# drapado/PINGS

Measured on AMD Instinct MI355X. Metric: raster fwd+bwd Mpix/s @1M Gaussians 1080p, higher is better.
Workload: dtype f32; 1 GPU; surfel rasteriser fwd+bwd, 1000000 Gaussians, 1920x1080, one view per GPU; gaussians=1000000, width=1920, height=1080

## Files before the change

### include/pings_hip.h

```cpp
#ifndef PINGS_HIP_H_
#define PINGS_HIP_H_

#include <stddef.h>
#include <stdint.h>

#if defined(__cplusplus)
#define PINGS_EXTERN_C extern "C"
#else
#define PINGS_EXTERN_C
#endif
#define PINGS_API PINGS_EXTERN_C __attribute__((visibility("default")))

#define PINGS_OK 0
#define PINGS_ERR_ARG 1
#define PINGS_ERR_HIP 2
#define PINGS_ERR_CAPACITY 3


#define PINGS_ABI_VERSION 11
PINGS_API int pings_abi_version(void);
PINGS_API const char* pings_last_error(void);

PINGS_API int pings_prof_enable(int on);
PINGS_API int pings_prof_only(const char* stage);
PINGS_API int pings_prof_report(char* buf, size_t cap);


PINGS_API size_t pings_ssim_partials_count(int planes, int H, int W);

PINGS_API int pings_ssim_forward(const float* img1, const float* img2, int planes, int H, int W,
                                 int train, float* out_mean, float* dm_dmu1,
                                 float* dm_dsigma1_sq, float* dm_dsigma12, float* partials,
                                 void* stream);

PINGS_API int pings_ssim_backward(const float* img1, const float* img2, int planes, int H, int W,
                                  const float* dL_dmean, const float* dm_dmu1,
                                  const float* dm_dsigma1_sq, const float* dm_dsigma12,
                                  float* dL_dimg1, void* stream);


#define PINGS_RASTER_SURFEL 0
#define PINGS_RASTER_3DGS 1
#define PINGS_RASTER_2DGS 2

typedef struct pings_raster_settings {
  int32_t image_height, image_width;
  int32_t mode;
  int32_t front_only;
  double tanfovx, tanfovy;
  double scale_modifier;
  const float* bg;
  const float* viewmatrix;
  const float* projmatrix;
  const float* projmatrix_raw;
  const float* prcppoint;
} pings_raster_settings;

PINGS_API int pings_raster_mark_visible(const float* positions, int N,
                                        const pings_raster_settings* s, uint8_t* present,
                                        void* stream);

PINGS_API size_t pings_raster_geom_bytes(int P, int image_height, int image_width);
PINGS_API size_t pings_raster_binning_bytes(int64_t num_instances, int image_height,
                                            int image_width);
PINGS_API size_t pings_raster_image_bytes(int image_height, int image_width);

PINGS_API int pings_raster_preprocess(const pings_raster_settings* s, int P, const float* means3D,
                                      const float* colors, const float* opacities,
                                      const float* scales, const float* rotations,
                                      void* geom_blob, int32_t* radii, int64_t* num_instances,
                                      int32_t* footprint_class, void* stream);
PINGS_API int pings_raster_preprocess_dyn(const pings_raster_settings* s, int P, const float* means3D,
                                          const float* colors, const float* opacities, const float* scales,
                                          const float* rotations, void* geom_blob, int32_t* radii,
                                          const int32_t* live_rows_dev, int dyn_rows,
                                          const int32_t* const* aux_dev, int aux_words, int32_t* aux_host,
                                          int64_t* num_instances, int32_t* footprint_class, void* stream);

PINGS_API int pings_raster_render(const pings_raster_settings* s, int P, int64_t num_instances,
                                  void* geom_blob, void* binning_blob, void* image_blob,
                                  float* out_color, float* out_normal,
                                  float* out_depth, float* out_alpha, void* per_gaussian,
                                  int footprint_class, void* stream);

PINGS_API size_t pings_raster_tile_sort_bytes(int64_t n, int32_t* block_pairs);
PINGS_API int pings_raster_tile_sort(const void* keys, int64_t n, int key_bytes, int bits, void* keys_sorted,
                                     uint32_t* values, void* scratch, int library, void* stream);

PINGS_API size_t pings_raster_scan_bytes(int64_t n);
PINGS_API int pings_raster_scan_u32(const void* in, int64_t n, int kind, int inclusive, uint32_t* out, void* temp,
                                    size_t temp_bytes, void* stream);

PINGS_API size_t pings_raster_backward_bytes(int P, int64_t num_instances);

PINGS_API int pings_raster_backward(const pings_raster_settings* s, int P, int64_t num_instances,
                                    const float* means3D, const float* colors,
                                    const float* opacities, const float* scales,
                                    const float* rotations, const void* geom_blob,
                                    const void* binning_blob, const void* image_blob,
                                    const float* out_color, const float* out_normal,
                                    const float* out_depth, const float* out_alpha,
                                    const float* dL_dcolor, const float* dL_dnormal,
                                    const float* dL_ddepth, const float* dL_dalpha,
                                    void* bwd_blob, float* dL_dmeans3D, float* dL_dmeans2D,
                                    float* dL_dcolors, float* dL_dopacities, float* dL_dscales,
                                    float* dL_drotations, float* dL_dtau, int footprint_class,
                                    void* stream);

PINGS_API int pings_raster_debug_lists(const void* binning_blob, int64_t num_instances,
                                       int image_height, int image_width, uint32_t* point_list,
                                       uint32_t* ranges_xy, void* stream);
PINGS_API int pings_raster_debug_image(const void* image_blob, int image_height, int image_width,
                                       float* final_T, uint32_t* n_contrib, void* stream);
PINGS_API int pings_raster_debug_occlusion(const void* geom_blob, int P, int image_height, int image_width,
                                           uint32_t* occ_bucket, uint16_t* occ_bsat, int32_t* occ_nb,
                                           void* stream);
PINGS_API int pings_raster_rank_bucket(const int32_t* ranks, int64_t n, int occ_nb, uint32_t nvalid,
                                       uint32_t* buckets);


PINGS_API size_t pings_raster2d_geom_bytes(int P, int image_height, int image_width);
PINGS_API size_t pings_raster2d_binning_bytes(int64_t num_instances, int image_height, int image_width);
PINGS_API size_t pings_raster2d_image_bytes(int image_height, int image_width);

PINGS_API int pings_raster2d_preprocess(const pings_raster_settings* s, int P, const float* means3D,
                                        const float* colors, const float* opacities, const float* scales,
                                        const float* rotations, void* geom_blob, int32_t* radii,
                                        const int32_t* live_rows_dev, int dyn_rows, const int32_t* const* aux_dev,
                                        int aux_words, int32_t* aux_host, int64_t* num_instances, void* stream);

PINGS_API int pings_raster2d_render(const pings_raster_settings* s, int P, int64_t num_instances, void* geom_blob,
                                    void* binning_blob, void* image_blob, float* out_color, float* out_allmap,
                                    void* stream);

PINGS_API size_t pings_raster2d_backward_bytes(int P, int64_t num_instances);

PINGS_API int pings_raster2d_backward(const pings_raster_settings* s, int P, int64_t num_instances,
                                      const float* scales, const float* rotations, const void* geom_blob,
                                      const void* binning_blob, const void* image_blob, const float* dL_dcolor,
                                      const float* dL_dallmap, void* bwd_blob, float* dL_dmeans3D,
                                      float* dL_dmeans2D, float* dL_dcolors, float* dL_dopacities,
                                      float* dL_dscales, float* dL_drotations, void* stream);

PINGS_API int pings_raster2d_debug_lists(const void* binning_blob, int64_t num_instances, int image_height,
                                         int image_width, uint32_t* point_list, uint32_t* ranges_xy, void* stream);
PINGS_API int pings_raster2d_debug_image(const void* image_blob, int image_height, int image_width, float* final_T,
                                         uint32_t* n_contrib, int32_t* median, void* stream);

typedef struct pings_knn_map {
  const int64_t* table;
  int64_t buffer_size;
  const float* neural_points;
  const int32_t* point_ts_create;
  const float* travel_dist;
  int32_t cur_ts;
  int32_t time_filtering;
  float diff_travel_dist_local;
  const uint8_t* free_mask;
  const uint8_t* valid_mask;
  int32_t use_free_mask, use_valid_mask;
  const int64_t* global2local;
  const int32_t* neighbor_dx;
  int32_t K;
  int32_t nn_k;
  float resolution;
  float max_valid_dist2;
  const void* compact;
  uint32_t compact_mask;
  const void* blocks;
  const void* block_records;
  const int32_t* blocks_ok;
  uint32_t block_mask;
} pings_knn_map;

PINGS_API size_t pings_knn_compact_entries(int64_t num_points);
PINGS_API int pings_knn_compact_build(const int64_t* table, int64_t buffer_size, void* compact,
                                      size_t entries, void* stream);

PINGS_API size_t pings_knn_blocks_entries(int64_t num_points);
PINGS_API int pings_knn_blocks_build(const pings_knn_map* m, int64_t num_points, int64_t num_timestamps,
                                     int32_t max_abs_dx, void* blocks, size_t entries, void* records,
                                     int32_t* status, void* stream);

PINGS_API int pings_knn_search(const pings_knn_map* m, const float* queries, int64_t B,
                               int64_t* idx, float* d2, int64_t* nn_counts, int64_t* global_idx,
                               void* stream);
PINGS_API int pings_knn_cells(const pings_knn_map* m, const float* queries, int64_t B, int64_t num_points, float* d2,
                              int64_t* idx, void* stream);

typedef struct pings_qf_tables {
  const float* geo_features;
  const float* color_features;
  int32_t Fg, Fc;
  const float* points;
  const float* orientations;
  const float* certainties;
  int32_t after_pgo;
  int32_t weighted_first;
} pings_qf_tables;

PINGS_API int pings_query_feature_forward(const pings_knn_map* m, const pings_qf_tables* t, const float* queries,
                                          int64_t B, float* geo_out, float* color_out, float* w_out,
                                          int64_t* idx_out, int64_t* gidx_out, int64_t* nn_counts,
                                          float* certainty, float* certainty_accum, const int32_t* query_ts,
                                          int32_t* ts_update, float* n_out, void* stream);
PINGS_API int pings_query_feature_accumulate(const int64_t* idx, const float* w, int64_t n_pairs, float* certainties,
                                             void* stream);

PINGS_API size_t pings_query_feature_scratch_bytes(int64_t B, int nn_k, int64_t rows);
PINGS_API int pings_query_feature_backward(const pings_qf_tables* t, const float* global_points,
                                           const float* queries, int64_t B, int nn_k, const int64_t* idx,
                                           const int64_t* gidx, const float* g_geo, const float* g_color,
                                           const float* g_n, const float* g_w, int64_t rows, void* scratch,
                                           float* g_x, float* g_geo_features, float* g_color_features,
                                           void* stream);

PINGS_API int pings_query_feature_double_backward(
    const pings_qf_tables* t, const float* global_points, const float* queries, int64_t B, int nn_k,
    const int64_t* idx, const int64_t* gidx, const float* g_geo, const float* g_color, const float* g_w,
    const float* gg_x, const float* gg_geo_features, const float* gg_color_features, int64_t rows, void* scratch,
    float* d_g_geo, float* d_g_color, float* d_g_n, float* d_g_w, float* d_x, float* d_geo_features,
    float* d_color_features, void* stream);

PINGS_API size_t pings_rows_scatter_add_scratch_bytes(int64_t n_pairs, int64_t rows);
PINGS_API int pings_rows_scatter_add(const int64_t* dst_row, int64_t n_pairs, const float* src, int64_t ld,
                                     int32_t F, const float* w, const int64_t* src_row, int64_t rows,
                                     void* scratch, float* out, void* stream);
PINGS_API size_t pings_rows_plan_bytes(int64_t n_pairs, int64_t rows);
PINGS_API int pings_rows_plan_build(const int64_t* dst_row, int64_t n_pairs, int64_t rows, void* plan, void* stream);
PINGS_API int pings_rows_plan_apply(const void* plan, int64_t n_pairs, int64_t rows, const float* src, int64_t ld,
                                    int32_t F, const float* w, float* out, void* stream);

typedef struct pings_sdf_decoder {
  const float* W1;
  const float* b1;
  const float* W2;
  const float* b2;
  int32_t hidden;
  int32_t feat_dim;
  float sdf_scale;
  int32_t weighted_first;
} pings_sdf_decoder;

PINGS_API int pings_sdf_forward(const pings_knn_map* m, const pings_sdf_decoder* dec,
                                const float* features, const float* points,
                                const float* orientations, const float* certainties,
                                int32_t after_pgo, const float* queries, int64_t B, float* sdf,
                                float* grad_x, int64_t* nn_counts, float* certainty,
                                int64_t* idx_out, float* w_out, float* sdf_std, int64_t* gidx_out,
                                void* stream);

PINGS_API int pings_sdf_plan(int nn_k, int feat_dim, int hidden, int weighted_first, int order, int misaligned,
                             int32_t* out);

typedef struct pings_color_decoder {
  const float* W1;
  const float* b1;
  const float* W2;
  const float* b2;
  int32_t hidden;
  int32_t feat_dim;
  int32_t channels;
  int32_t weighted_first;
} pings_color_decoder;
PINGS_API int pings_color_forward(const pings_color_decoder* dec, const float* features, int64_t rows,
                                  const float* points, const float* orientations, int32_t after_pgo,
                                  const float* queries, int64_t B, const int64_t* idx, int32_t nn_k, float* color,
                                  float* jac, void* stream);

PINGS_API size_t pings_sdf_backward_scratch_bytes(int64_t B, int nn_k, int feat_dim, int hidden,
                                                  int64_t feature_rows);
// ... 617 lines not shown
```

### pings_amd/_abi.py

```python
from __future__ import annotations

import ctypes as C

ABI_VERSION = 11

RASTER_SURFEL, RASTER_3DGS, RASTER_2DGS = 0, 1, 2
HEAD_COLOR, HEAD_SEMANTIC = 0, 1
REG_SINGULAR, REG_ILL_CONDITIONED, REG_NONFINITE = 1, 2, 4
REG_F_NORMALS, REG_F_DIV_GRAD, REG_F_WEIGHTED = 1, 2, 4
REG_COLOR_PHOTO, REG_COLOR_CONSIST = 1, 2
MC_ALLOW_DEGENERATE, MC_ASCENT = 1, 2
ADAMW_MAX_JOBS, ADAMW_CHUNK = 48, 4096
EVAL_VIEW_RECORD, EVAL_PAIR_RECORD = 9, 12
EVAL_EXTENT = 1
LOOP_MAX_R, LOOP_MAX_S, LOOP_MAX_D = 32, 128, 16
LOOP_MAX_Q, LOOP_MAX_C = 16, 65536
LIDAR_MAX_CAMS, LIDAR_MAX_LIDARS = 8, 8
CAMFRONT_MAX_MAPS, CAMFRONT_TILE_W, CAMFRONT_TILE_H = 32, 128, 32
CAMFRONT_RGB_U8, CAMFRONT_RGB_F32, CAMFRONT_NORMAL, CAMFRONT_DEPTH, CAMFRONT_SKY = 0, 1, 2, 3, 4
CAMFRONT_FIT_RECORD, CAMFRONT_MIN_FIT = 5, 100
CAMFRONT_FULL = 2
TSDF_BLOCK = 8
TSDF_EXTENT, TSDF_TABLE_FULL = 1, 2

# ... 33 lines not shown

class SdfDecoder(C.Structure):
    _fields_ = [("W1", C.c_void_p), ("b1", C.c_void_p), ("W2", C.c_void_p), ("b2", C.c_void_p),
                ("hidden", C.c_int32), ("feat_dim", C.c_int32), ("sdf_scale", C.c_float),
                ("weighted_first", C.c_int32)]


class ColorDecoder(C.Structure):
    _fields_ = [("W1", C.c_void_p), ("b1", C.c_void_p), ("W2", C.c_void_p), ("b2", C.c_void_p),
                ("hidden", C.c_int32), ("feat_dim", C.c_int32), ("channels", C.c_int32),
                ("weighted_first", C.c_int32)]


class MlpJob(C.Structure):
    _fields_ = [("x", C.c_void_p), ("IN", C.c_int32), ("OUT", C.c_int32), ("W1", C.c_void_p), ("b1", C.c_void_p),
                ("W2", C.c_void_p), ("b2", C.c_void_p), ("y", C.c_void_p), ("dL_dy", C.c_void_p), ("dL_dx", C.c_void_p),
                ("dL_dW1", C.c_void_p), ("dL_db1", C.c_void_p), ("dL_dW2", C.c_void_p), ("dL_db2", C.c_void_p)]


class SpawnParams(C.Structure):
    _fields_ = [("n", C.c_int), ("k", C.c_int), ("scale_dim", C.c_int), ("surfel", C.c_int),
                ("color_residual", C.c_int), ("alpha_filter_on", C.c_int), ("scale_filter_on", C.c_int),
                ("displacement_range", C.c_float), ("unit_scale", C.c_float), ("max_scale", C.c_float),
                ("scale_filter_thr", C.c_float)]


class GatherJob(C.Structure):
    _fields_ = [("src", C.c_void_p), ("dst", C.c_void_p), ("row_bytes", C.c_int64), ("rows", C.c_int64)]


class ImageLossParams(C.Structure):
    _fields_ = [("H", C.c_int), ("W", C.c_int), ("v_min", C.c_int), ("v_max", C.c_int), ("depth_min", C.c_float),
                ("depth_max", C.c_float), ("min_accu_alpha", C.c_float), ("inverse_depth", C.c_int),
                ("consist_mode", C.c_int)]


class RegLoopArgs(C.Structure):
    _fields_ = [("n", C.c_int64), ("flags", C.c_int32), ("iter", C.c_int32), ("trace_cap", C.c_int32),
                ("min_grad", C.c_float), ("max_grad", C.c_float), ("max_std", C.c_float), ("gm_dist", C.c_float),
                ("gm_grad", C.c_float), ("lm_lambda", C.c_float)] + \
               [(k, C.c_void_p) for k in ("src", "cur", "sdf", "grad", "std", "mask", "label", "normals", "valid",
                                          "part", "T", "delta", "record", "trace")]


class RegColorArgs(C.Structure):
    _fields_ = [("src_color", C.c_void_p), ("color_pred", C.c_void_p), ("color_jac", C.c_void_p),
                ("channels", C.c_int32), ("mode", C.c_int32), ("photo_weight", C.c_float), ("photo_part", C.c_void_p)]


class GaussLossArgs(C.Structure):
    _fields_ = [("P", C.c_int64), ("Na", C.c_int64), ("cap", C.c_int64), ("R", C.c_int32), ("ncols", C.c_int32),
                ("scale_cols", C.c_int32), ("flags", C.c_int32), ("min_alpha", C.c_float),
                ("contrib_thr", C.c_float), ("shift_range", C.c_float), ("grad_min", C.c_float),
                ("grad_max", C.c_float), ("inv_voxel_pow", C.c_float), ("n_inject", C.c_int64)] + \
               [(n, vp) for n in ("alpha_all", "visible", "contrib", "free_mask", "xyz", "rot", "scale", "alpha", "seed",
                                  "inject_idx", "randn", "keys", "part", "meta", "idx", "normal", "queries", "label",
                                  "sdf", "grad", "nn", "valid", "losses", "counts", "g", "ds", "v", "dn", "dq",
                                  "d_xyz", "d_rot", "d_scale", "d_alpha", "d_alpha_all")]


class SdfHvpArgs(C.Structure):
    _fields_ = [("W1", vp), ("b1", vp), ("W2", vp), ("b2", vp), ("H", C.c_int32), ("F", C.c_int32),
                ("scale", C.c_float), ("after_pgo", C.c_int32), ("features", vp), ("points", vp),
                ("orientations", vp), ("gpoints", vp), ("queries", vp), ("B", C.c_int64), ("nnk", C.c_int32),
                ("idx", vp), ("gidx", vp), ("v", vp), ("ds", vp), ("grad_x", vp), ("out", vp)]


class SdfLossArgs(C.Structure):
    _fields_ = [("B", C.c_int64), ("cap", C.c_int64), ("k", C.c_int32), ("C", C.c_int32), ("d", C.c_int32),
                ("flags", C.c_int32), ("sigma", C.c_float), ("eik_band", C.c_float), ("col_band", C.c_float)] + \
               [(n, vp) for n in ("coord", "label", "weight", "color_label", "w", "s", "c", "g", "idx", "xsel", "meta",
                                  "part", "sdf_pred", "losses", "counts", "gl", "g_pred", "d_s", "d_g", "d_c")]


class AdamwJob(C.Structure):
    _fields_ = [("p", vp), ("g", vp), ("m", vp), ("v", vp), ("n", C.c_int64)] + \
               [(n, C.c_float) for n in ("decay", "beta1", "beta2", "one_minus_beta1", "one_minus_beta2", "step_size",
                                         "bc2_sqrt", "eps")]


class CameraPoseArgs(C.Structure):
    _fields_ = [(n, vp) for n in ("R", "T", "projection_matrix", "world_view_transform", "full_proj_transform",
                                  "camera_center", "cam_trans_delta", "cam_rot_delta", "out")] + \
               [(n, C.c_int64) for n in ("R_s0", "R_s1", "T_s", "proj_s0", "proj_s1", "wvt_s0", "wvt_s1", "fpt_s0",
                                         "fpt_s1", "center_s")] + [("converged_threshold", C.c_double)]


class PoolSampleArgs(C.Structure):
    _fields_ = [("P", C.c_int64)] + \
               [(n, C.c_int32) for n in ("surface_sample_n", "free_front_n", "free_behind_n", "color_channels",
                                         "dist_weight_on", "behind_dropoff_on", "sem_is_i64", "reserved")] + \
               [(n, C.c_double) for n in ("surface_sample_range", "free_sample_begin_ratio", "free_sample_end_dist",
                                          "dist_weight_scale", "max_range")] + \
               [(n, vp) for n in ("points", "normal", "sem", "color", "noise_surface", "noise_front", "noise_behind",
                                  "coord", "sdf_label", "weight", "out_normal", "out_sem", "out_color")]


class PoolAppendArgs(C.Structure):
    _fields_ = [(n, C.c_int64) for n in ("n", "m", "capacity")] + \
               [(n, C.c_int32) for n in ("frame_id", "color_channels", "pose_is_f64", "reserved")] + \
               [(n, vp) for n in ("pose", "coord", "sdf_label", "weight", "sem", "color", "normal", "global_coord_pool",
                                  "sdf_label_pool", "weight_pool", "time_pool", "sem_label_pool", "color_pool",
                                  "normal_label_pool")]


class PoolSelectArgs(C.Structure):
    _fields_ = [(n, C.c_int64) for n in ("n", "capacity")] + \
               [(n, C.c_int32) for n in ("color_channels", "pose_is_f64", "select_all", "reserved")] + \
               [("thr", C.c_double)] + \
               [(n, vp) for n in ("pose", "coord", "sdf_label", "color", "normal", "scratch", "out_points", "out_color",
                                  "out_normal")]


class LidarCam(C.Structure):
    _fields_ = [(n, vp) for n in ("image", "K", "T", "keys", "src", "l0", "l1", "l2", "l3")] + \
               [("H", C.c_int32), ("W", C.c_int32)]


class CamfrontMap(C.Structure):
    _fields_ = [(n, vp) for n in ("src", "l0", "l1", "l2", "l3")] + \
               [(n, C.c_int64) for n in ("stride_c", "stride_y", "stride_x")] + \
               [(n, C.c_int32) for n in ("H", "W", "kind", "reserved")]


SIGNATURES = {
    "pings_abi_version": (i32, []),
    "pings_last_error": (C.c_char_p, []),
    "pings_prof_enable": (i32, [i32]),
    "pings_prof_only": (i32, [C.c_char_p]),
    "pings_prof_report": (i32, [C.c_char_p, sz]),
    "pings_ssim_partials_count": (sz, [i32, i32, i32]),
    "pings_ssim_forward": (i32, [vp, vp, i32, i32, i32, i32, vp, vp, vp, vp, vp, vp]),
    "pings_ssim_backward": (i32, [vp, vp, i32, i32, i32, vp, vp, vp, vp, vp, vp]),
    "pings_raster_mark_visible": (i32, [vp, i32, C.POINTER(RasterSettings), vp, vp]),
    "pings_raster_geom_bytes": (sz, [i32, i32, i32]),
    "pings_raster_binning_bytes": (sz, [i64, i32, i32]),
    "pings_raster_image_bytes": (sz, [i32, i32]),
    "pings_raster_preprocess": (i32, [C.POINTER(RasterSettings), i32, vp, vp, vp, vp, vp, vp, vp, C.POINTER(i64),
                                      C.POINTER(i32), vp]),
    "pings_raster_preprocess_dyn": (i32, [C.POINTER(RasterSettings), i32, vp, vp, vp, vp, vp, vp, vp, vp, i32,
                                          C.POINTER(vp), i32, C.POINTER(i32), C.POINTER(i64), C.POINTER(i32), vp]),
    "pings_raster_render": (i32, [C.POINTER(RasterSettings), i32, i64, vp, vp, vp, vp, vp, vp, vp, vp, i32, vp]),
    "pings_raster_tile_sort_bytes": (sz, [i64, C.POINTER(i32)]),
    "pings_raster_tile_sort": (i32, [vp, i64, i32, i32, vp, vp, vp, i32, vp]),
    "pings_raster_scan_bytes": (sz, [i64]),
    "pings_raster_scan_u32": (i32, [vp, i64, i32, i32, vp, vp, sz, vp]),
    "pings_raster_backward_bytes": (sz, [i32, i64]),
    "pings_raster_backward": (i32, [C.POINTER(RasterSettings), i32, i64, vp, vp, vp, vp, vp, vp, vp, vp, vp, vp, vp, vp,
                                    vp, vp, vp, vp, vp, vp, vp, vp, vp, vp, vp, vp, i32, vp]),
    "pings_raster_debug_lists": (i32, [vp, i64, i32, i32, vp, vp, vp]),
    "pings_raster_debug_image": (i32, [vp, i32, i32, vp, vp, vp]),
    "pings_raster_debug_occlusion": (i32, [vp, i32, i32, i32, vp, vp, C.POINTER(C.c_int32), vp]),
    "pings_raster_rank_bucket": (i32, [vp, i64, i32, C.c_uint32, vp]),
    "pings_raster2d_geom_bytes": (sz, [i32, i32, i32]),
    "pings_raster2d_binning_bytes": (sz, [i64, i32, i32]),
    "pings_raster2d_image_bytes": (sz, [i32, i32]),
    "pings_raster2d_preprocess": (i32, [C.POINTER(RasterSettings), i32, vp, vp, vp, vp, vp, vp, vp, vp, i32,
                                        C.POINTER(vp), i32, C.POINTER(i32), C.POINTER(i64), vp]),
    "pings_raster2d_render": (i32, [C.POINTER(RasterSettings), i32, i64, vp, vp, vp, vp, vp, vp]),
    "pings_raster2d_backward_bytes": (sz, [i32, i64]),
    "pings_raster2d_backward": (i32, [C.POINTER(RasterSettings), i32, i64, vp, vp, vp, vp, vp, vp, vp, vp, vp, vp, vp,
                                      vp, vp, vp, vp]),
    "pings_raster2d_debug_lists": (i32, [vp, i64, i32, i32, vp, vp, vp]),
    "pings_raster2d_debug_image": (i32, [vp, i32, i32, vp, vp, vp, vp]),
    "pings_knn_compact_entries": (sz, [i64]),
    "pings_knn_compact_build": (i32, [vp, i64, vp, sz, vp]),
    "pings_knn_blocks_entries": (sz, [i64]),
    "pings_knn_blocks_build": (i32, [C.POINTER(KnnMap), i64, i64, i32, vp, sz, vp, vp, vp]),
    "pings_knn_search": (i32, [C.POINTER(KnnMap), vp, i64, vp, vp, vp, vp, vp]),
    "pings_knn_cells": (i32, [C.POINTER(KnnMap), vp, i64, i64, vp, vp, vp]),
    "pings_query_feature_forward": (i32, [C.POINTER(KnnMap), C.POINTER(QfTables), vp, i64, vp, vp, vp, vp, vp, vp, vp,
                                          vp, vp, vp, vp, vp]),
    "pings_query_feature_accumulate": (i32, [vp, vp, i64, vp, vp]),
    "pings_query_feature_scratch_bytes": (sz, [i64, i32, i64]),
    "pings_query_feature_backward": (i32, [C.POINTER(QfTables), vp, vp, i64, i32, vp, vp, vp, vp, vp, vp, i64, vp, vp,
                                           vp, vp, vp]),
    "pings_query_feature_double_backward": (i32, [C.POINTER(QfTables), vp, vp, i64, i32, vp, vp, vp, vp, vp, vp, vp, vp,
                                                  i64, vp, vp, vp, vp, vp, vp, vp, vp, vp]),
    "pings_rows_scatter_add_scratch_bytes": (sz, [i64, i64]),
    "pings_rows_scatter_add": (i32, [vp, i64, vp, i64, i32, vp, vp, i64, vp, vp, vp]),
    "pings_rows_plan_bytes": (sz, [i64, i64]),
    "pings_rows_plan_build": (i32, [vp, i64, i64, vp, vp]),
    "pings_rows_plan_apply": (i32, [vp, i64, i64, vp, i64, i32, vp, vp, vp]),
    "pings_sdf_forward": (i32, [C.POINTER(KnnMap), C.POINTER(SdfDecoder), vp, vp, vp, vp, i32, vp, i64, vp, vp, vp, vp,
                                vp, vp, vp, vp, vp]),
    "pings_sdf_plan": (i32, [i32, i32, i32, i32, i32, i32, C.POINTER(C.c_int32)]),
    "pings_color_forward": (i32, [C.POINTER(ColorDecoder), vp, i64, vp, vp, i32, vp, i64, vp, i32, vp, vp, vp]),
    "pings_sdf_backward_scratch_bytes": (sz, [i64, i32, i32, i32, i64]),
    "pings_sdf_double_backward": (i32, [C.POINTER(SdfDecoder), vp, i64, vp, vp, vp, i32, vp, i64, i32, vp, vp, vp, vp,
                                        vp, vp, vp, vp, vp, vp, vp]),
    "pings_sdf_backward": (i32, [C.POINTER(SdfDecoder), vp, i64, vp, vp, i32, vp, i64, i32, vp, vp, vp, vp, vp, vp, vp,
                                 vp, vp, vp]),
    "pings_mlp_backward_scratch_bytes": (sz, [i32, i32, i32]),
    "pings_mlp_forward": (i32, [vp, i64, i32, i32, i32, vp, vp, vp, vp, vp, vp]),
    "pings_mlp_backward": (i32, [vp, vp, i64, i32, i32, i32, vp, vp, vp, vp, vp, vp, vp, vp, vp, vp]),
    "pings_mlp_double_backward_supported": (i32, [i32, i32, i32]),
    "pings_mlp_double_backward": (i32, [vp, vp, vp, i64, i32, i32, i32, vp, vp, vp, vp, vp, vp, vp, vp]),
    "pings_mlp_forward_grouped": (i32, [C.POINTER(MlpJob), i32, i64, vp]),
    "pings_mlp_forward_grouped_dyn": (i32, [C.POINTER(MlpJob), i32, i64, vp, vp]),
    "pings_mlp_backward_grouped_scratch_bytes": (sz, [C.POINTER(MlpJob), i32]),
    "pings_mlp_backward_grouped": (i32, [C.POINTER(MlpJob), i32, i64, vp, vp]),
    "pings_exposure_forward": (i32, [vp, vp, vp, i64, vp, vp]),
    "pings_exposure_backward_scratch_bytes": (sz, []),
    "pings_exposure_backward": (i32, [vp, vp, vp, i64, vp, vp, vp, vp, vp]),
    "pings_stencil_points": (i32, [vp, i64, f32, i32, vp, vp]),
    "pings_stencil_gradient": (i32, [vp, vp, i64, f32, i32, vp, vp]),
    "pings_stencil_gradient_backward": (i32, [vp, i64, f32, i32, vp, vp, vp]),
    "pings_spawn_gather": (i32, [i32, vp, vp, vp, vp, vp, vp, i32, vp, i32, vp, i32, i32, i32, vp, vp, vp, vp, vp, vp,
                                 vp, vp]),
    "pings_spawn_gather_dyn": (i32, [i32, vp, vp, vp, vp, vp, vp, vp, i32, vp, i32, vp, i32, i32, i32, vp, vp, vp, vp,
                                     vp, vp, vp, vp]),
    "pings_spawn_plan_dyn": (i32, [C.POINTER(SpawnParams), vp, vp, vp, vp, vp, vp, vp, vp, vp]),
    "pings_spawn_forward_dyn": (i32, [C.POINTER(SpawnParams), vp, vp, vp, vp, vp, vp, vp, vp, vp, vp, vp, vp, vp, vp,
                                      vp, vp, vp, vp, vp, vp, vp]),
    "pings_spawn_gather_backward": (i32, [i32, vp, vp, i32, i32, vp, i32, i32, vp, vp, vp]),
    "pings_spawn_plan_scratch_bytes": (sz, [i64]),
    "pings_spawn_plan": (i32, [C.POINTER(SpawnParams), vp, vp, vp, vp, vp, vp, vp]),
    "pings_spawn_forward": (i32, [C.POINTER(SpawnParams), vp, vp, vp, vp, vp, vp, vp, vp, vp, vp, vp, vp, vp, vp, vp,
                                  vp, vp, vp, vp]),
    "pings_spawn_backward": (i32, [C.POINTER(SpawnParams), vp, vp, vp, vp, vp, vp, vp, vp, vp, vp, vp, vp, vp, vp, vp,
                                   vp, vp, vp, vp, vp, vp]),
    "pings_voxel_downsample_scratch_bytes": (sz, [i64]),
    "pings_voxel_downsample": (i32, [vp, i64, f32, vp, vp, C.POINTER(i64), vp]),
    "pings_voxel_downsample_min_value": (i32, [vp, vp, i64, f32, vp, vp, C.POINTER(i64), vp]),
    "pings_map_prune_mask": (i32, [i64, vp, i64, i32, vp, vp, f32, f32, vp, vp, vp]),
    "pings_map_adjust": (i32, [i64, vp, vp, vp, vp, i32, vp, i32, i64, vp, vp]),
    "pings_map_rehash": (i32, [vp, vp, i64, f32, i64, vp, vp, vp]),
    "pings_map_update_scratch_bytes": (sz, [i64, i64]),
    "pings_map_update": (i32, [vp, vp, i64, f64, i64, vp, i64, vp, i32, f32, i32, vp, vp, vp, vp, vp, vp, vp, vp, vp,
                               vp, vp, C.POINTER(i64), vp]),
    "pings_map_reset_local_scratch_bytes": (sz, [i64]),
    "pings_map_reset_local": (i32, [i64, vp, vp, vp, vp, i32, i32, i32, f32, i32, vp, i32, f64, f64, vp, vp, vp, vp, vp,
                                    C.POINTER(i64), vp]),
    "pings_mask_rows_scratch_bytes": (sz, [i64]),
    "pings_mask_rows": (i32, [vp, i64, vp, vp, C.POINTER(i64), vp]),
    "pings_gather_rows_multi": (i32, [C.POINTER(GatherJob), i32, vp, vp]),
    "pings_gather_rows": (i32, [vp, i64, vp, i64, vp, vp]),
    "pings_scatter_rows": (i32, [vp, i64, vp, i64, vp, vp]),
    "pings_depth2normal_forward": (i32, [vp, vp, vp, i32, i32, f32, f32, f32, f32, f32, vp, vp]),
    "pings_depth2normal_backward_scratch_bytes": (sz, [i32, i32]),
    "pings_depth2normal_backward": (i32, [vp, vp, vp, i32, i32, f32, f32, f32, f32, f32, vp, vp, vp, vp]),
    "pings_image_losses_scratch_bytes": (sz, []),
    "pings_image_losses_forward": (i32, [C.POINTER(ImageLossParams), vp, vp, vp, vp, vp, vp, vp, vp, vp, vp, vp, vp]),
    "pings_image_losses_backward": (i32, [C.POINTER(ImageLossParams), vp, vp, vp, vp, vp, vp, vp, vp, vp, vp, vp, vp,
                                          vp, vp, vp, vp]),
    "pings_head_reduce": (i32, [vp, vp, i64, i32, i32, i32, vp, vp, vp]),
    "pings_reg_normal_equations_scratch_bytes": (sz, []),
    "pings_reg_normal_equations": (i32, [vp, vp, vp, vp, i64, vp, vp, vp]),
    "pings_reg_solve": (i32, [vp, f32, vp, vp, vp]),
    "pings_reg_solve_checked": (i32, [vp, f32, vp, vp, vp, C.POINTER(i32), vp]),
    "pings_reg_partials": (i32, [i64]),
    "pings_reg_transform": (i32, [C.POINTER(RegLoopArgs), vp]),
    "pings_reg_assemble": (i32, [C.POINTER(RegLoopArgs), vp]),
    "pings_reg_step": (i32, [C.POINTER(RegLoopArgs), vp]),
    "pings_reg_assemble_color": (i32, [C.POINTER(RegLoopArgs), C.POINTER(RegColorArgs), vp]),
    "pings_reg_read_record": (i32, [vp, vp, vp]),
    "pings_gauss_loss_select": (i32, [C.POINTER(GaussLossArgs), vp]),
    "pings_gauss_loss_prepare": (i32, [C.POINTER(GaussLossArgs), vp]),
    "pings_gauss_loss_reduce": (i32, [C.POINTER(GaussLossArgs), vp]),
    "pings_gauss_loss_backward_rows": (i32, [C.POINTER(GaussLossArgs), vp]),
    "pings_gauss_loss_backward_scatter": (i32, [C.POINTER(GaussLossArgs), vp]),
    "pings_sdf_hvp_x": (i32, [C.POINTER(SdfHvpArgs), vp]),
    "pings_sdf_loss_select": (i32, [C.POINTER(SdfLossArgs), vp]),
    "pings_sdf_loss_reduce": (i32, [C.POINTER(SdfLossArgs), vp]),
    "pings_sdf_loss_backward": (i32, [C.POINTER(SdfLossArgs), vp]),
    "pings_sdf_loss_partials": (i32, [i64, i64]),
    "pings_mc_scratch_bytes": (sz, [i64, i64, i64]),
    "pings_mc_count": (i32, [vp, vp, i64, i64, i64, f32, i32, vp, C.POINTER(i64), vp]),
    "pings_mc_emit": (i32, [vp, vp, i64, i64, i64, f32, i32, vp, i64, i64, vp, vp, vp, vp]),
    "pings_mesh_weld_scratch_bytes": (sz, [i64, i64]),
    "pings_mesh_weld": (i32, [vp, i64, vp, i64, vp, vp, vp, vp, vp, C.POINTER(i64), vp]),
    "pings_mesh_clusters_scratch_bytes": (sz, [i64]),
    "pings_mesh_clusters": (i32, [vp, i64, i64, vp, vp, vp, C.POINTER(i64), vp]),
    "pings_mesh_drop_small_scratch_bytes": (sz, [i64]),
    "pings_mesh_drop_small": (i32, [vp, i64, vp, vp, i64, vp, vp, C.POINTER(i64), vp]),
    "pings_mesh_vertex_normals_scratch_bytes": (sz, [i64, i64]),
    "pings_mesh_vertex_normals": (i32, [vp, i64, vp, i64, vp, vp, vp]),
    "pings_mesh_compact_vertices_scratch_bytes": (sz, [i64, i64]),
    "pings_mesh_compact_vertices": (i32, [vp, i64, vp, i64, vp, vp, vp, vp, vp, C.POINTER(i64), vp]),
    "pings_adamw_step": (i32, [C.POINTER(AdamwJob), i32, C.POINTER(i32), vp]),
    "pings_eval_view_metrics_scratch_bytes": (sz, [i64]),
    "pings_eval_view_metrics": (i32, [vp, vp, i32, i64, vp, vp, vp, f32, f32, f32, i32, vp, vp, vp, vp]),
    "pings_eval_backproject_scratch_bytes": (sz, [i64]),
    "pings_eval_backproject": (i32, [vp, vp, vp, i32, i32, C.POINTER(f64), C.POINTER(f64), f64, f32, i32, vp, vp, vp,
                                     vp, vp]),
    "pings_eval_voxel_scratch_bytes": (sz, [i64]),
    "pings_eval_voxel_centroids": (i32, [vp, i64, vp, f64, vp, vp, vp, vp, vp]),
    "pings_eval_nn_scratch_bytes": (sz, [i64]),
    "pings_eval_nn_build": (i32, [vp, i64, vp, f64, vp, vp, vp]),
    "pings_eval_nn_query": (i32, [vp, i64, vp, vp, i64, f64, f64, vp, vp, vp]),
    "pings_eval_pair_reduce": (i32, [vp, i64, vp, vp, i64, vp, f64, f64, vp, vp, vp]),
    "pings_camera_update_pose": (i32, [C.POINTER(CameraPoseArgs), vp]),
    "pings_camera_set_pose": (i32, [vp, i32, i64, i64, vp, i64, i64, vp, vp]),
    "pings_pool_sample": (i32, [C.POINTER(PoolSampleArgs), vp]),
    "pings_pool_draw": (i32, [C.POINTER(GatherJob), i32, vp, i64, vp, i64, vp, i64, vp, i64, i64, vp, vp]),
    "pings_pool_ts_range": (i32, [vp, i32, i64, vp, vp]),
    "pings_pool_transform": (i32, [i64, vp, vp, i32, vp, i32, i64, vp, vp]),
    "pings_pool_window_scratch_bytes": (sz, [i64]),
    "pings_pool_window_count": (i32, [vp, i64, vp, f32, i32, vp, C.POINTER(i64), vp]),
    "pings_pool_window": (i32, [vp, i64, vp, f32, i32, vp, vp, i64, vp]),
    "pings_pool_append": (i32, [C.POINTER(PoolAppendArgs), vp]),
    "pings_pool_discard_mark": (i32, [vp, i64, i64, vp, vp, vp]),
    "pings_pool_compact_scratch_bytes": (sz, [i64]),
    "pings_pool_compact_count": (i32, [vp, i64, i64, vp, C.POINTER(i64), vp]),
    "pings_pool_compact": (i32, [C.POINTER(GatherJob), i32, vp, i64, vp, vp]),
    "pings_pool_select_scratch_bytes": (sz, [i64]),
# ... 41 lines not shown
```

### pings_amd/csrc/raster_bwd.hip

```cpp
#include <hipcub/hipcub.hpp>

#include <algorithm>
#include <type_traits>

#include "raster_common.hpp"

namespace pings {
namespace raster {

constexpr int BATCH = 64;
constexpr uint32_t LONG_TILES_MAX = 2048;
constexpr uint32_t DEAD_ROW = 0xFFFFFFFFu;

template <int MODE>
__device__ __forceinline__ void blend_bwd_tile_body(
    BParams p, const uint2* __restrict__ ranges, const uint32_t* __restrict__ point_list,
    const float4* __restrict__ rec, const uint32_t* __restrict__ gval, const float* __restrict__ final_T,
    const uint32_t* __restrict__ n_contrib, const float* __restrict__ out_depth, const float* __restrict__ dL_dcolor,
    const float* __restrict__ dL_dnormal, const float* __restrict__ dL_ddepth, const float* __restrict__ dL_dalpha,
    const float* __restrict__ inst_w, const uint32_t* __restrict__ cidx, float* __restrict__ rows,
    const uint32_t* __restrict__ tile_order) {
  __shared__ float4 sA[BATCH], sB[BATCH], sC[BATCH], sD[BATCH];
  __shared__ uint32_t sRow[BATCH];
  __shared__ float4 sG[BATCH][4];
  __shared__ uint8_t sList[BATCH];

  const int lane = threadIdx.x;
  const int tile = (int)tile_order[blockIdx.x];
  const int tx = tile % p.gx, ty = tile / p.gx;
  const int pix_x = tx * TILE + (lane & 7), pix_y0 = ty * TILE + (lane >> 3);
  const f2 pixf_x = {(float)pix_x, (float)(pix_x + 8)};
  const float pixf_y[2] = {(float)pix_y0, (float)(pix_y0 + 8)};
  const float tileX0 = (float)(tx * TILE), tileY0 = (float)(ty * TILE);
  const size_t HW = (size_t)p.W * p.H;

  f2 rx = {0.f, 0.f};
  float ry[2] = {0.f, 0.f};
  if (MODE == MODE_SURFEL) {
    const float cxp = (p.prcp ? p.prcp[0] : 0.5f) * (float)p.W - 0.5f;
    const float cyp = (p.prcp ? p.prcp[1] : 0.5f) * (float)p.H - 0.5f;
    rx = f2{(pixf_x.x - cxp) / p.fx, (pixf_x.y - cxp) / p.fx};
#pragma unroll
    for (int r = 0; r < 2; ++r) ry[r] = (pixf_y[r] - cyp) / p.fy;
  }

  const uint2 range = ranges[tile];
  uint32_t last[2][2];
  f2 T[2], gC0[2], gC1[2], gC2[2], gN0[2], gN1[2], gN2[2], gD[2];
  f2 Bs[2];
  uint32_t lmax = 0;
#pragma unroll
  for (int r = 0; r < 2; ++r) {
    T[r] = f2{1.f, 1.f};
    gC0[r] = gC1[r] = gC2[r] = gN0[r] = gN1[r] = gN2[r] = gD[r] = Bs[r] = f2{0.f, 0.f};
#pragma unroll
    for (int h = 0; h < 2; ++h) {
      last[r][h] = 0;
      const int pix_y = pix_y0 + 8 * r, pix_xh = pix_x + 8 * h;
      if (pix_xh < p.W && pix_y < p.H) {
        const size_t pix_id = (size_t)pix_y * p.W + pix_xh;
        last[r][h] = n_contrib[pix_id];
        const float T_final = final_T[pix_id];
        T[r][h] = T_final;
        float c0 = 0.f, c1 = 0.f, c2 = 0.f;
        if (dL_dcolor) {
          c0 = dL_dcolor[pix_id];
          c1 = dL_dcolor[HW + pix_id];
          c2 = dL_dcolor[2 * HW + pix_id];
        }
        gC0[r][h] = c0;
        gC1[r][h] = c1;
        gC2[r][h] = c2;
        float gA = dL_dalpha ? dL_dalpha[pix_id] : 0.f;
        const float gDo = dL_ddepth ? dL_ddepth[pix_id] : 0.f;
        if (MODE == MODE_SURFEL) {
          if (dL_dnormal) {
            gN0[r][h] = dL_dnormal[pix_id];
            gN1[r][h] = dL_dnormal[HW + pix_id];
            gN2[r][h] = dL_dnormal[2 * HW + pix_id];
          }
          const float A = 1.0f - T_final;
          if (A > DEPTH_ALPHA_EPS) {
            gD[r][h] = gDo / A;
            gA -= gDo * out_depth[pix_id] / A;
          }
        } else {
          gD[r][h] = gDo;
        }
        Bs[r][h] = ((p.bg[0] * c0 + p.bg[1] * c1) + p.bg[2] * c2) - gA;
      }
      lmax = max(lmax, last[r][h]);
    }
  }
#pragma unroll
  for (int off = 32; off > 0; off >>= 1) lmax = max(lmax, (uint32_t)__shfl_xor((int)lmax, off, 64));
  const int max_last = __builtin_amdgcn_readfirstlane((int)lmax);
  const int red_slot = red16_lane_slot(lane);
  const bool red_store = (lane & 12) == 0;
  const float red_scale = (red_slot == G_CONX || red_slot == G_CONZ) ? 0.5f : 1.0f;

  const int nbatch = ceil_div(max_last, BATCH);
  for (int b = nbatch - 1; b >= 0; --b) {
    const int start = b * BATCH;
    const int n = min(BATCH, max_last - start);
    __syncthreads();
    bool hit = false;
    if (lane < n) {
      const uint32_t slot = point_list[range.x + start + lane];
      const uint32_t g = gval[slot];
      const float4 ra = rec[4 * (size_t)g + 0];
      const float4 rb = rec[4 * (size_t)g + 1];
      sA[lane] = ra;
      sB[lane] = rb;
      sC[lane] = rec[4 * (size_t)g + 2];
      if (MODE == MODE_SURFEL) sD[lane] = rec[4 * (size_t)g + 3];
      const bool live = inst_w[slot] > 0.f;
      sRow[lane] = live ? cidx[slot] : DEAD_ROW;
      if (live) hit = quadrant_mask(ra.x, ra.y, ra.z, rb.x, rb.y, rb.z, tileX0, tileY0) != 0u;
    }
    const unsigned long long bal = __ballot(hit);
    if (hit) sList[__builtin_amdgcn_mbcnt_hi((uint32_t)(bal >> 32), __builtin_amdgcn_mbcnt_lo((uint32_t)bal, 0u))] = (uint8_t)lane;
    const int cnt = __popcll(bal);
    {
      float4* z = &sG[0][0];
      const float4 zero = make_float4(0.f, 0.f, 0.f, 0.f);
      for (int e = lane; e < BATCH * 4; e += 64) z[e] = zero;
    }
    __syncthreads();

    int i0 = cnt > 0 ? (int)sList[cnt - 1] : 0;
    int i1 = cnt > 1 ? (int)sList[cnt - 2] : 0;
    float4 a0 = sA[i0], b0 = sB[i0], c0 = sC[i0], n0 = make_float4(0.f, 0.f, 0.f, 0.f);
    float4 a1, b1, c1, n1 = n0;
    if (MODE == MODE_SURFEL) n0 = sD[i0];
    auto trip = [&](const float4& ca, const float4& cb, const float4& cc, const float4& cn, const int j)
                    __attribute__((always_inline)) {
      const uint32_t idx = (uint32_t)(start + j);
      const f2 dx = f2s(ca.x) - pixf_x;
      const f2 p0 = f2s(-0.5f) * ((f2s(cb.x) * dx) * dx);
      const f2 pxy = f2s(cb.y) * dx;
      f2 Gs[2], raw[2], alpha[2];
      float dyv[2];
      bool valid[2][2];
      bool any_v = false;
#pragma unroll
      for (int r = 0; r < 2; ++r) {
        const float dy = ca.y - pixf_y[r];
        dyv[r] = dy;
        const f2 power = (p0 - f2s(0.5f * (cb.z * dy * dy))) - pxy * f2s(dy);
        Gs[r] = f2{__expf(power.x), __expf(power.y)};
        raw[r] = f2s(ca.z) * Gs[r];
        alpha[r] = f2{fminf(ALPHA_MAX, raw[r].x), fminf(ALPHA_MAX, raw[r].y)};
        valid[r][0] = idx < last[r][0] && (power.x <= 0.0f) && (alpha[r].x >= ALPHA_MIN);
        valid[r][1] = idx < last[r][1] && (power.y <= 0.0f) && (alpha[r].y >= ALPHA_MIN);
        any_v = any_v || valid[r][0] || valid[r][1];
      }
      if (!__any(any_v)) return;

      {
#pragma clang fp contract(fast)
      f2 v2[16];
      if (MODE != MODE_SURFEL) v2[G_NX] = v2[G_NY] = v2[G_NZ] = v2[G_Q] = v2[G_ZLO] = v2[G_ZHI] = f2{0.f, 0.f};
      const float zlo = ca.w - cb.w, zhi = ca.w + cb.w;
      const float zlo_m = fminf(zlo, zhi);
      const f2 cxdx = f2s(cb.x) * dx;
#pragma unroll
      for (int r = 0; r < 2; ++r) {
        const bool first = r == 0;
        auto acc = [&](int q, f2 x) { v2[q] = first ? x : v2[q] + x; };
        const f2 av = sel2(valid[r][0], valid[r][1], alpha[r], f2{0.f, 0.f});
        const f2 one_m = f2s(1.0f) - av;
        const f2 inv_one_m = {__builtin_amdgcn_rcpf(one_m.x), __builtin_amdgcn_rcpf(one_m.y)};
        const f2 Tn = T[r] * inv_one_m;
        const f2 w = av * Tn;
        f2 sdot = (f2s(cc.x) * gC0[r] + f2s(cc.y) * gC1[r]) + f2s(cc.z) * gC2[r];
        acc(G_R, gC0[r] * w);
        acc(G_G, gC1[r] * w);
        acc(G_B, gC2[r] * w);
        if (MODE == MODE_SURFEL) {
          sdot += (f2s(cn.x) * gN0[r] + f2s(cn.y) * gN1[r]) + f2s(cn.z) * gN2[r];
          const f2 den = fma2(f2s(cn.x), rx, f2s(fmaf(cn.y, ry[r], cn.z)));
          const bool hit0 = den.x < -DEN_EPS, hit1 = den.y < -DEN_EPS;
          const f2 inv_den = {__builtin_amdgcn_rcpf(den.x), __builtin_amdgcn_rcpf(den.y)};
          const f2 d0 = sel2(hit0, hit1, f2s(cc.w) * inv_den, f2s(ca.w));
          const f2 d = {__builtin_amdgcn_fmed3f(d0.x, zlo_m, zhi), __builtin_amdgcn_fmed3f(d0.y, zlo_m, zhi)};
          sdot = fma2(d, gD[r], sdot);
          const f2 gd = gD[r] * w;
          const bool lo0 = d0.x < zlo, lo1 = d0.y < zlo, hi0 = d0.x > zhi, hi1 = d0.y > zhi;
          const bool mid0 = !lo0 && !hi0, mid1 = !lo1 && !hi1;
          const f2 zero = {0.f, 0.f};
          acc(G_ZLO, sel2(lo0, lo1, gd, zero));
          acc(G_ZHI, sel2(hi0, hi1, gd, zero));
          const f2 gq = sel2(mid0 && hit0, mid1 && hit1, gd * inv_den, zero);
          acc(G_Q, gq);
          acc(G_PZ, sel2(mid0 && !hit0, mid1 && !hit1, gd, zero));
          const f2 gden = -gq * d0;
          v2[G_NX] = fma2(gden, rx, first ? gN0[r] * w : fma2(gN0[r], w, v2[G_NX]));
          v2[G_NY] = fma2(gden, f2s(ry[r]), first ? gN1[r] * w : fma2(gN1[r], w, v2[G_NY]));
          v2[G_NZ] = fma2(gN2[r], w, first ? gden : v2[G_NZ] + gden);
        } else {
          sdot = fma2(f2s(ca.w), gD[r], sdot);
          acc(G_PZ, gD[r] * w);
        }
        f2 dLda = sdot - Bs[r];
        Bs[r] = fma2(av, dLda, Bs[r]);
        dLda = dLda * Tn;
        dLda = sel2(valid[r][0] && raw[r].x <= ALPHA_MAX, valid[r][1] && raw[r].y <= ALPHA_MAX, dLda, f2{0.f, 0.f});
        acc(G_OPAC, Gs[r] * dLda);
        const f2 dLp = raw[r] * dLda;
        const f2 qx = cxdx + f2s(cb.y * dyv[r]), qy = pxy + f2s(cb.z * dyv[r]);
        const f2 ux = dLp * qx, uy = dLp * qy;
        acc(G_MX, -ux);
        acc(G_MY, -uy);
        acc(G_CONX, ux * qx);
        acc(G_CONY, ux * qy);
        acc(G_CONZ, uy * qy);
        T[r] = Tn;
      }
      const float tot = wave_reduce16_swap<MODE != MODE_SURFEL>(v2, lane) * red_scale;
      if (red_store) reinterpret_cast<float*>(&sG[j][0])[red_slot] = tot;
      }
    };
    for (int jj = cnt - 1; jj >= 0; jj -= 2) {
      {
        const int j = i0;
        a1 = sA[i1]; b1 = sB[i1]; c1 = sC[i1];
        if (MODE == MODE_SURFEL) n1 = sD[i1];
        i0 = (int)sList[jj > 1 ? jj - 2 : 0];
        trip(a0, b0, c0, n0, j);
      }
      if (jj == 0) break;
      {
        const int j = i1;
        a0 = sA[i0]; b0 = sB[i0]; c0 = sC[i0];
        if (MODE == MODE_SURFEL) n0 = sD[i0];
        i1 = (int)sList[jj > 2 ? jj - 3 : 0];
        trip(a1, b1, c1, n1, j);
      }
    }
    __syncthreads();
    for (int e = lane; e < n * 4; e += 64) {
      const int j = e >> 2, part = e & 3;
      if (sRow[j] != DEAD_ROW) reinterpret_cast<float4*>(rows)[(size_t)sRow[j] * 4 + part] = sG[j][part];
    }
  }
}

struct GradFill {
  float* ptr[6];
  size_t count[6];
};
typedef float v4f __attribute__((ext_vector_type(4)));
__device__ inline void grad_fill_part(const GradFill& f, uint32_t part, uint32_t nparts) {
  const size_t tid = (size_t)part * blockDim.x + threadIdx.x, nthreads = (size_t)nparts * blockDim.x;
#pragma unroll
  for (int a = 0; a < 6; ++a) {
    float* const p = f.ptr[a];
    const size_t n = f.count[a];
    const size_t head = min(n, (size_t)((16u - (uint32_t)(reinterpret_cast<uintptr_t>(p) & 15u)) & 15u) >> 2);
    const size_t nvec = (n - head) >> 2;
    v4f* const body = reinterpret_cast<v4f*>(p + head);
    for (size_t i = tid; i < nvec; i += nthreads) __builtin_nontemporal_store(v4f{0.f, 0.f, 0.f, 0.f}, body + i);
    const size_t tail = head + 4 * nvec;
    if (tid < head) p[tid] = 0.f;
    if (tid < n - tail) p[tail + tid] = 0.f;
  }
}

template <int MODE>
__global__ __launch_bounds__(64, 3) void blend_bwd_tile_kernel(
    BParams p, const uint2* __restrict__ ranges, const uint32_t* __restrict__ point_list,
    const float4* __restrict__ rec, const uint32_t* __restrict__ gval, const float* __restrict__ final_T,
    const uint32_t* __restrict__ n_contrib, const float* __restrict__ out_depth, const float* __restrict__ dL_dcolor,
    const float* __restrict__ dL_dnormal, const float* __restrict__ dL_ddepth, const float* __restrict__ dL_dalpha,
    const float* __restrict__ inst_w, const uint32_t* __restrict__ cidx, float* __restrict__ rows,
    const uint32_t* __restrict__ tile_order, uint32_t num_tiles, GradFill fill) {
  if (blockIdx.x >= num_tiles) {
    grad_fill_part(fill, blockIdx.x - num_tiles, gridDim.x - num_tiles);
    return;
  }
  blend_bwd_tile_body<MODE>(p, ranges, point_list, rec, gval, final_T, n_contrib, out_depth, dL_dcolor, dL_dnormal,
                            dL_ddepth, dL_dalpha, inst_w, cidx, rows, tile_order);
}

__global__ __launch_bounds__(64) void tile_max_contrib_kernel(int W, int H, int gx, const uint32_t* __restrict__ n_contrib,
                                                              uint32_t* __restrict__ work) {
  const int tile = blockIdx.x, lane = threadIdx.x;
  const int tx = tile % gx, ty = tile / gx;
  uint32_t m = 0;
#pragma unroll
  for (int r = 0; r < 4; ++r) {
    const int x = tx * TILE + (lane & 15), y = ty * TILE + 4 * r + (lane >> 4);
    if (x < W && y < H) m = max(m, n_contrib[(size_t)y * W + x]);
  }
#pragma unroll
  for (int off = 32; off > 0; off >>= 1) m = max(m, (uint32_t)__shfl_xor((int)m, off, 64));
  if (lane == 0) work[tile] = m;
}

template <int CTRL, int ROW_MASK>
__device__ inline float dpp_f(float old, float v) {
  return __builtin_bit_cast(float, __builtin_amdgcn_update_dpp(__builtin_bit_cast(int, old), __builtin_bit_cast(int, v),
                                                                CTRL, ROW_MASK, 0xf, false));
}

__device__ inline float wave_incl_scan_mul(float x) {
  x *= dpp_f<0x111, 0xf>(1.f, x);
  x *= dpp_f<0x112, 0xf>(1.f, x);
  x *= dpp_f<0x114, 0xf>(1.f, x);
  x *= dpp_f<0x118, 0xf>(1.f, x);
  x *= dpp_f<0x142, 0xa>(1.f, x);
  x *= dpp_f<0x143, 0xc>(1.f, x);
  return x;
}

__device__ inline float wave_incl_scan_add(float x) {
  x += dpp_f<0x111, 0xf>(0.f, x);
  x += dpp_f<0x112, 0xf>(0.f, x);
  x += dpp_f<0x114, 0xf>(0.f, x);
  x += dpp_f<0x118, 0xf>(0.f, x);
  x += dpp_f<0x142, 0xa>(0.f, x);
  x += dpp_f<0x143, 0xc>(0.f, x);
  return x;
}

__device__ inline float wave_shr1(float x, float first) { return dpp_f<0x138, 0xf>(first, x); }

template <int G>
__device__ inline float grp_incl_scan_mul(float x) {
  x *= dpp_f<0x111, 0xf>(1.f, x);
  x *= dpp_f<0x112, 0xf>(1.f, x);
  x *= dpp_f<0x114, 0xf>(1.f, x);
  x *= dpp_f<0x118, 0xf>(1.f, x);
  if (G >= 32) x *= dpp_f<0x142, 0xa>(1.f, x);
  if (G >= 64) x *= dpp_f<0x143, 0xc>(1.f, x);
  return x;
}
template <int G>
__device__ inline float grp_incl_scan_add(float x) {
  x += dpp_f<0x111, 0xf>(0.f, x);
  x += dpp_f<0x112, 0xf>(0.f, x);
  x += dpp_f<0x114, 0xf>(0.f, x);
  x += dpp_f<0x118, 0xf>(0.f, x);
  if (G >= 32) x += dpp_f<0x142, 0xa>(0.f, x);
  if (G >= 64) x += dpp_f<0x143, 0xc>(0.f, x);
  return x;
}
template <int G>
__device__ inline float grp_shr1(float x, float first, int lane) {
  if (G == 16) return dpp_f<0x111, 0xf>(first, x);
  const float y = dpp_f<0x138, 0xf>(first, x);
  return (G == 32 && lane == 32) ? first : y;
}

#ifdef PINGS_BWD_STATS
#define STATS_PARAMS , unsigned long long& st_dead, unsigned long long& st_any, unsigned long long& st_exec, unsigned long long& st_valid
#define STATS_ARGS , st_dead, st_any, st_exec, st_valid
#else
#define STATS_PARAMS
#define STATS_ARGS
#endif

template <int MODE, int G, int NPIX>
__device__ inline void scan_pixels(float4 (*sPix)[4], int lane, int pix0, int e, int min_e, const float4& a,
                                   const float4& b, const float4& c, const float4& nn, float (&v)[16] STATS_PARAMS) {
  constexpr int NG = 64 / G;
  const int grp = lane / G;
  const float zlo = a.w - b.w, zhi = a.w + b.w;
  for (int pp0 = 0; pp0 < NPIX; pp0 += NG) {
    const int pp = pix0 + pp0 + grp;
    const float4 s0 = sPix[pp][0];
    const int last_p = (int)__float_as_uint(s0.z);
    if (!__any(last_p > min_e)) {
#ifdef PINGS_BWD_STATS
      st_dead += NG;
#endif
      continue;
    }
    const float4 s1 = sPix[pp][1], s2 = sPix[pp][2], s3 = sPix[pp][3];
    const float T_p = s0.x, R_p = s0.y, coefT = s0.w;
    const float dx = a.x - s2.w;
    const float dy = a.y - s3.x;
    const float p0 = -0.5f * (b.x * dx * dx);
    const float pxy = b.y * dx;
    const float power = (p0 - 0.5f * (b.z * dy * dy)) - pxy * dy;
    const float Gs = __expf(power);
    const float raw = a.z * Gs;
    const float alpha = fminf(ALPHA_MAX, raw);
    const bool valid = (e < last_p) && (power <= 0.0f) && (alpha >= ALPHA_MIN);
#ifdef PINGS_BWD_STATS
    if (!__any(valid)) st_any += NG; else { st_exec += NG; st_valid += (unsigned)__popcll(__ballot(valid)); }
#endif
    if (!__any(valid)) continue;
    const float av = valid ? alpha : 0.f;
    const float P_in = grp_incl_scan_mul<G>(1.0f - av);
    const float P_ex = grp_shr1<G>(P_in, 1.0f, lane);
    const float inv_P = __builtin_amdgcn_rcpf(P_in);
    const float Tn = T_p * inv_P;
    const float inv_one_m = P_ex * inv_P;
    const float w = av * Tn;
    float S_in;
    {
#pragma clang fp contract(fast)
    float sdot = (c.x * s1.x + c.y * s1.y) + c.z * s1.z;
    v[G_R] = fmaf(s1.x, w, v[G_R]);
    v[G_G] = fmaf(s1.y, w, v[G_G]);
    v[G_B] = fmaf(s1.z, w, v[G_B]);
    if (MODE == MODE_SURFEL) {
      sdot += (nn.x * s2.x + nn.y * s2.y) + nn.z * s2.z;
      const float den = (nn.x * s3.y + nn.y * s3.z) + nn.z;
      const bool hit = den < -DEN_EPS;
      const float inv_den = __builtin_amdgcn_rcpf(den);
      const float d0 = hit ? c.w * inv_den : a.w;
      const float d = fminf(fmaxf(d0, zlo), zhi);
      sdot = fmaf(d, s1.w, sdot);
      const float gd = s1.w * w;
      const bool lo = d0 < zlo, hi = d0 > zhi;
      const bool mid = !lo && !hi;
      v[G_ZLO] += lo ? gd : 0.f;
      v[G_ZHI] += hi ? gd : 0.f;
      const float gq = (mid && hit) ? gd * inv_den : 0.f;
      v[G_Q] += gq;
      v[G_PZ] += (mid && !hit) ? gd : 0.f;
      const float gden = -gq * d0;
      v[G_NX] += fmaf(gden, s3.y, s2.x * w);
      v[G_NY] += fmaf(gden, s3.z, s2.y * w);
      v[G_NZ] += s2.z * w + gden;
    } else {
      sdot = fmaf(a.w, s1.w, sdot);
      v[G_PZ] = fmaf(s1.w, w, v[G_PZ]);
    }
    const float ws = w * sdot;
    S_in = grp_incl_scan_add<G>(ws);
    const float R_l = R_p + grp_shr1<G>(S_in, 0.f, lane);
    float dLda = fmaf(Tn, sdot, (coefT - R_l) * inv_one_m);
// ... 515 lines not shown
  if (owner) {
    if (!GROUP_SUM) sum_partials<PART_AHEAD>(partials, q, qb, G);
    gaussian_row<MODE>(p, (int)gidx_sorted[r], true, G, means3D, scales, rotations, dL_dmeans3D, dL_dmeans2D,
                       dL_dcolors, dL_dopacities, dL_dscales, dL_drotations, tau);
  }
  store_tau_partial(tau, tau_partials);
}

template <int MODE>
__global__ __launch_bounds__(256, 4) void gaussian_bwd_index_kernel(
    BParams p, const float* __restrict__ means3D, const float* __restrict__ scales,
    const float* __restrict__ rotations, const uint4* __restrict__ rect, const uint32_t* __restrict__ rank_of,
    const uint32_t* __restrict__ tiles_sorted, const uint32_t* __restrict__ pair_off,
    const float* __restrict__ partials, float* __restrict__ dL_dmeans3D, float* __restrict__ dL_dmeans2D, float* __restrict__ dL_dcolors,
    float* __restrict__ dL_dopacities, float* __restrict__ dL_dscales,
    float* __restrict__ dL_drotations, float* __restrict__ tau_partials) {
  const int g = blockIdx.x * blockDim.x + threadIdx.x;
  float tau[6] = {0.f, 0.f, 0.f, 0.f, 0.f, 0.f};
  if (g < p.P) {
    uint32_t n_tiles = 0u, qa = 0u, qb = 0u;
    if (rect[g].w != 0u) {
      const uint32_t rank = rank_of[g];
      n_tiles = tiles_sorted[rank];
      qa = pair_off[rank];
      qb = pair_off[rank + 1];
    }
    float G[16];
#pragma unroll
    for (int k = 0; k < 16; ++k) G[k] = 0.f;
    sum_partials<1>(partials, qa, qb, G);
    gaussian_row<MODE>(p, g, n_tiles > 0 && qb > qa, G, means3D, scales, rotations, dL_dmeans3D, dL_dmeans2D,
                       dL_dcolors, dL_dopacities, dL_dscales, dL_drotations, tau);
  }
  store_tau_partial(tau, tau_partials);
}

__global__ __launch_bounds__(256) void tau_reduce_kernel(const float* __restrict__ partials,
                                                          const uint32_t* __restrict__ npairs, int nblocks_all,
                                                          float* __restrict__ dL_dtau) {
  const int nblocks = npairs ? (int)((*npairs + 255u) / 256u) : nblocks_all;
  __shared__ double sRed[4][6];
  double s[6] = {0, 0, 0, 0, 0, 0};
  for (int i = threadIdx.x; i < nblocks; i += 256) {
#pragma unroll
    for (int k = 0; k < 6; ++k) s[k] += (double)partials[(size_t)i * 6 + k];
  }
#pragma unroll
  for (int k = 0; k < 6; ++k) {
#pragma unroll
    for (int off = 32; off > 0; off >>= 1) s[k] += __shfl_down(s[k], off, 64);
    if ((threadIdx.x & 63) == 0) sRed[threadIdx.x >> 6][k] = s[k];
  }
  __syncthreads();
  if (threadIdx.x < 6)
    dL_dtau[threadIdx.x] = (float)(((sRed[0][threadIdx.x] + sRed[1][threadIdx.x]) + sRed[2][threadIdx.x]) + sRed[3][threadIdx.x]);
}

}
}

using namespace pings::raster;

PINGS_API int pings_raster_backward(const pings_raster_settings* s, int P, int64_t I,
                                    const float* means3D, const float* colors,
                                    const float* opacities, const float* scales,
                                    const float* rotations, const void* geom_blob,
                                    const void* binning_blob, const void* image_blob,
                                    const float* out_color, const float* out_normal,
                                    const float* out_depth, const float* out_alpha,
                                    const float* dL_dcolor, const float* dL_dnormal,
                                    const float* dL_ddepth, const float* dL_dalpha,
                                    void* bwd_blob, float* dL_dmeans3D, float* dL_dmeans2D,
                                    float* dL_dcolors, float* dL_dopacities, float* dL_dscales,
                                    float* dL_drotations, float* dL_dtau, int footprint_class,
                                    void* stream) {
  BParams bp;
  if (int e = fill_camera(s, P, bp)) return e;
  PINGS_ARG_CHECK(dL_dtau != nullptr, "null dL_dtau");
  hipStream_t st = pings::as_stream(stream);
  if (P == 0) {
    PINGS_HIP_CHECK(hipMemsetAsync(dL_dtau, 0, 6 * sizeof(float), st));
    return PINGS_OK;
  }
  PINGS_ARG_CHECK(P > 0 && means3D && colors && opacities && scales && rotations && geom_blob &&
                      binning_blob && image_blob && out_depth && bwd_blob && dL_dmeans3D &&
                      dL_dmeans2D && dL_dcolors && dL_dopacities && dL_dscales && dL_drotations,
                  "null pointer");
  PINGS_ARG_CHECK(I >= 0 && I < (int64_t)0x7FFFFFF0, "instance count out of range");
  (void)out_color; (void)out_normal; (void)out_alpha;
  const RasterKnobs knobs = read_knobs();
  const int num_tiles = bp.gx * bp.gy;
  const BlendPlan plan = blend_plan(knobs, footprint_class, I, num_tiles);
  GeomState gs = carve_geom(const_cast<void*>(geom_blob), P, num_tiles);
  BinState bs = carve_binning(const_cast<void*>(binning_blob), I, num_tiles, knobs.blend_seg);
  ImageState im = carve_image(const_cast<void*>(image_blob), bp.W, bp.H);
  BwdState bw = carve_bwd(bwd_blob, P, I);
  const dim3 block(256);
  const RowRanges rr{P, gs.offsets_sorted, gs.tiles_sorted, bw.cidx};

  TileOrderJob order_job;
  if (I > 0) {
    pings::prof::Scope ps("tile_order", st);
    const bool fwd_left_it = plan.fwd == BlendPlan::FWD_TILE;
    if (!fwd_left_it) {
      hipLaunchKernelGGL(tile_max_contrib_kernel, dim3(num_tiles), dim3(64), 0, st, bp.W, bp.H, bp.gx, im.n_contrib,
                         bs.tile_work);
      PINGS_LAUNCH_CHECK();
    }
    order_job.work = fwd_left_it ? bs.tile_maxc : bs.tile_work;
    order_job.num_tiles = num_tiles;
    order_job.order = bs.tile_order + num_tiles;
    order_job.n_long = bs.tile_order + 2 * (size_t)num_tiles;
    order_job.long_thr = plan.long_thr;
    order_job.long_max = LONG_TILES_MAX;
  }
  {
    pings::prof::Scope ps("live_scan", st);
    if (I > 0 && plan.bwd_scan) {
      if (int e = raster_scan_pop(bs.inst_qmask, I + 1, bw.cidx, bw.temp, bw.temp_bytes, knobs.library_scan, order_job, st))
        return e;
    } else if (I > 0) {
      if (int e = raster_scan_live(bs.inst_w, I + 1, bw.cidx, bw.temp, bw.temp_bytes, knobs.library_scan, order_job, st))
        return e;
    } else {
      PINGS_HIP_CHECK(hipMemsetAsync(bw.cidx, 0, 2 * sizeof(uint32_t), st));
    }
    if (int e = raster_scan_chunks(rr, bw.pair_off, bw.pair_owner, bw.temp, bw.temp_bytes, knobs.library_scan, st))
      return e;
  }
  const bool by_rank = !plan.bwd_scan;
  GradFill fill;
  {
    float* const grads[6] = {dL_dmeans3D, dL_dmeans2D, dL_dcolors, dL_dopacities, dL_dscales, dL_drotations};
    const size_t per[6] = {3, 3, 3, 1, 3, 4};
    for (int a = 0; a < 6; ++a) { fill.ptr[a] = grads[a]; fill.count[a] = per[a] * (size_t)P; }
  }
  const bool fill_in_blend = by_rank && I > 0 && knobs.grad_fill_wgs > 0;
  if (I > 0) {
    pings::prof::Scope ps("blend_bwd", st);
    const uint32_t* order = bs.tile_order + num_tiles;
    with_mode(s->mode, [&](auto m) {
      constexpr int M = m();
      if (plan.bwd_scan) {
        const uint32_t* n_long = bs.tile_order + 2 * (size_t)num_tiles;
        const unsigned grid_s = (unsigned)(num_tiles + 3 * std::min<long long>(num_tiles, LONG_TILES_MAX));
        hipLaunchKernelGGL((blend_bwd_scan_kernel<M>), dim3(grid_s), dim3(256), 0, st, bp, bs.ranges,
                           bs.point_list, gs.rec, bs.gval, im.final_T, im.n_contrib, out_depth, dL_dcolor, dL_dnormal,
                           dL_ddepth, dL_dalpha, bs.inst_qmask, bw.cidx, bw.rows, order, n_long);
      } else {
        const unsigned fill_wgs = fill_in_blend ? knobs.grad_fill_wgs : 0u;
        hipLaunchKernelGGL((blend_bwd_tile_kernel<M>), dim3((unsigned)num_tiles + fill_wgs), dim3(64), 0, st, bp,
                           bs.ranges, bs.point_list, gs.rec, bs.gval, im.final_T, im.n_contrib, out_depth, dL_dcolor,
                           dL_dnormal, dL_ddepth, dL_dalpha, bs.inst_w, bw.cidx, bw.rows, order, (uint32_t)num_tiles,
                           fill);
      }
    });
    PINGS_LAUNCH_CHECK();
  }
  {
    pings::prof::Scope ps("row_chunk_sum", st);
    hipLaunchKernelGGL(row_chunk_sum_kernel, dim3(knobs.rowsum_wgs), block, 0, st, rr, bw.pair_off, bw.pair_owner,
                       bw.rows, bw.partials);
    PINGS_LAUNCH_CHECK();
  }
  const int nblocks = pings::ceil_div(P, 256);
  {
    pings::prof::Scope ps_g("gaussian_bwd", st);
    if (by_rank && !fill_in_blend) {
      const unsigned fill_grid = (unsigned)std::min<size_t>(2048, pings::ceil_div<size_t>((size_t)P * 17, 4 * 256));
      hipLaunchKernelGGL(grad_zero_kernel, dim3(fill_grid), block, 0, st, fill);
      PINGS_LAUNCH_CHECK();
    }
    with_mode(s->mode, [&](auto m) {
      if (by_rank) {
        const auto chain = knobs.chain_sum_lanes ? gaussian_bwd_rank_kernel<m(), false> : gaussian_bwd_rank_kernel<m(), true>;
        hipLaunchKernelGGL(chain, dim3((unsigned)pings::ceil_div<size_t>(bw.np_max, 256)), block,
                           0, st, bp, means3D, scales, rotations, gs.gidx_sorted, bw.pair_off, bw.pair_owner,
                           bw.partials, dL_dmeans3D, dL_dmeans2D, dL_dcolors, dL_dopacities, dL_dscales, dL_drotations,
                           bw.tau_partials);
      } else
        hipLaunchKernelGGL(gaussian_bwd_index_kernel<m()>, dim3(nblocks), block, 0, st, bp, means3D, scales, rotations,
                           gs.rect, gs.rank_of, gs.tiles_sorted, bw.pair_off, bw.partials, dL_dmeans3D, dL_dmeans2D,
                           dL_dcolors, dL_dopacities, dL_dscales, dL_drotations, bw.tau_partials);
    });
    PINGS_LAUNCH_CHECK();
    hipLaunchKernelGGL(tau_reduce_kernel, dim3(1), block, 0, st, bw.tau_partials,
                       by_rank ? (const uint32_t*)(bw.pair_off + P) : (const uint32_t*)nullptr, nblocks, dL_dtau);
    PINGS_LAUNCH_CHECK();
  }
  return PINGS_OK;
}

#ifdef PINGS_BWD_STATS
PINGS_API int pings_debug_bwd_stats(unsigned long long* out8, int reset) {
  PINGS_HIP_CHECK(hipDeviceSynchronize());
  PINGS_HIP_CHECK(hipMemcpyFromSymbol(out8, HIP_SYMBOL(pings::raster::g_bwd_stats), 64));
  if (reset) {
    unsigned long long z[8] = {0};
    PINGS_HIP_CHECK(hipMemcpyToSymbol(HIP_SYMBOL(pings::raster::g_bwd_stats), z, 64));
  }
  return PINGS_OK;
}
#endif
```

### pings_amd/csrc/raster_common.hpp

```cpp
#pragma once
#include <cstdlib>
#include <type_traits>

#include "common.hpp"

namespace pings {
namespace raster {

constexpr int TILE = 16;
constexpr int BLOCK = TILE * TILE;
constexpr float NEAR_Z = 0.2f;
constexpr float LOWPASS = 0.3f;
constexpr float ALPHA_MAX = 0.99f;
constexpr float ALPHA_MIN = 1.0f / 255.0f;
constexpr float T_EPS = 1e-4f;
constexpr float DEPTH_ALPHA_EPS = 1e-10f;
constexpr float DEN_EPS = 1e-6f;
constexpr uint32_t CULLED_KEY = 0xFFFFFFFFu;
constexpr int DS_NB = 1 << 20;
constexpr uint32_t DS_LIMIT = 4096u;
constexpr int DS_SHARDS = 64;
constexpr int DS_KMIN = 2 * DS_SHARDS, DS_SHIFT = DS_KMIN + 1, DS_FLAG = DS_KMIN + 2, DS_HEAD = DS_KMIN + 8;
constexpr int STAT_SHARDS = 256;
constexpr int STAT_PAIRS = 0, STAT_VISIBLE = STAT_SHARDS, STAT_KEPT = 2 * STAT_SHARDS;
constexpr int STAT_BMAX = 3 * STAT_SHARDS, STAT_WORDS = STAT_BMAX + 1, STAT_RETRY_WORDS = STAT_WORDS - STAT_KEPT;
static_assert((STAT_SHARDS & (STAT_SHARDS - 1)) == 0, "the shard of a wave is its number modulo a power of two");
constexpr float OCC_THR = 9.5f;
constexpr float OCC_FIX = 4096.f;
constexpr uint16_t OCC_ALL = 0xFFFFu;

constexpr int MODE_SURFEL = 0;
constexpr int MODE_3DGS = 1;
constexpr int RECT_TIGHT = 0, RECT_3SIGMA = 1, RECT_ELLIPSE = 2;

constexpr int GRAD_ROW = 16;
constexpr int CH = 64;
enum GradSlot {
  G_MX = 0, G_MY = 1, G_CONX = 2, G_CONY = 3, G_CONZ = 4, G_OPAC = 5,
  G_R = 6, G_G = 7, G_B = 8, G_NX = 9, G_NY = 10, G_NZ = 11, G_Q = 12, G_PZ = 13,
  G_ZLO = 14, G_ZHI = 15
};

struct FrameSummary {
  uint32_t overflow, pad0;
  unsigned long long stats[3];
  int32_t aux[8];
  uint32_t seq;
  uint32_t pad;
};

struct GeomState {
  float4* rec;
  uint4* rect;
  uint32_t *depth_key, *depth_key_sorted, *gidx, *gidx_sorted;
  uint32_t* rank_of;
  uint32_t *tiles_sorted, *offsets_sorted;
  uint32_t* occ_bucket;
  uint16_t* occ_bsat;
  unsigned long long* occ_mask;
  uint32_t* nvalid;
  uint32_t* occ_bmax;
  uint32_t* ds_head;
  uint32_t *ds_cnt, *ds_fill, *ds_off;
  char* zero_begin; size_t zero_bytes;
  size_t ds_words;
  uint32_t* ds_idx;
  unsigned long long* stats;
  FrameSummary* summary;
  int occ_nb, occ_words;
  char* temp;
  size_t temp_bytes;
  size_t total;
};

struct BinState {
  uint32_t *tile_key, *tile_key_sorted, *gval, *point_list;
  uint32_t* slot_val;
  uint2* ranges;
  float* inst_w;
  uint8_t* inst_qmask;
  float* inst_wq;
  uint32_t* inst_cntq;
  uint32_t* inst_cnt;
  uint32_t* tile_order;
  uint32_t* tile_work;
  uint32_t* tile_maxc;
  uint32_t seg_max_units;
  uint32_t *seg_head, *seg_unit_tile, *seg_unit_seg, *seg_tile_unit0;
  float *seg_P, *seg_slab;
  uint16_t* seg_rel;
  uint32_t* seg_nrel;
  char* temp;
  size_t temp_bytes;
  size_t total;
};

struct ImageState {
  float* final_T;
  uint32_t* n_contrib;
  size_t total;
};

struct KParams {
  int P, W, H, gx, gy;
  int front_only;
  float occ_amin;
  int rect_rule;
  float fx, fy, limx, limy, scale_mod;
  const float* view;
  const float* proj_raw;
  const float* bg;
  const float* prcp;
  const int32_t* live;
  int dyn_rows;
};

struct BParams {
  int P, W, H, gx, gy;
  int front_only;
  float fx, fy, limx, limy, scale_mod;
  const float* view;
  const float* proj_raw;
  const float* bg;
  const float* prcp;
};

template <typename Params>
int fill_camera(const pings_raster_settings* s, int P, Params& kp) {
  PINGS_ARG_CHECK(s != nullptr, "null settings");
  PINGS_ARG_CHECK(s->image_height > 0 && s->image_width > 0, "empty image");
  PINGS_ARG_CHECK(s->image_height < 65536 * TILE / 16 && s->image_width < 65536, "image too large");
  PINGS_ARG_CHECK(s->mode == PINGS_RASTER_SURFEL || s->mode == PINGS_RASTER_3DGS, "unknown mode");
  PINGS_ARG_CHECK(s->viewmatrix && s->projmatrix_raw && s->bg, "null camera pointer");
  PINGS_ARG_CHECK(s->tanfovx > 0 && s->tanfovy > 0, "non-positive tanfov");
  kp.P = P;
  kp.W = s->image_width;
  kp.H = s->image_height;
  kp.gx = ceil_div(kp.W, TILE);
  kp.gy = ceil_div(kp.H, TILE);
  kp.front_only = s->front_only;
  kp.fx = (float)((double)kp.W / (2.0 * s->tanfovx));
  kp.fy = (float)((double)kp.H / (2.0 * s->tanfovy));
  kp.limx = (float)(1.3 * s->tanfovx);
  kp.limy = (float)(1.3 * s->tanfovy);
  kp.scale_mod = (float)s->scale_modifier;
  kp.view = s->viewmatrix;
  kp.proj_raw = s->projmatrix_raw;
  kp.bg = s->bg;
  kp.prcp = s->prcppoint;
  return PINGS_OK;
}

template <typename F>
decltype(auto) with_mode(int mode, F&& f) {
  if (mode == PINGS_RASTER_SURFEL) return f(std::integral_constant<int, MODE_SURFEL>{});
  return f(std::integral_constant<int, MODE_3DGS>{});
}

struct RasterKnobs {
  enum Bwd { BWD_AUTO, BWD_PIXEL, BWD_SCAN };
  int blend_ppl = 0;
  Bwd blend_bwd = BWD_AUTO;
  uint32_t blend_seg = 512u;
  bool seg_reuse = true;
  uint32_t bwd_long = 3072u;
  bool occlusion = true;
  bool library_sort = false;
  bool library_tile_sort = false;
  bool library_scan = false;
  float occ_amin = 0.15f;
  bool occ_walk_lanes = false;
  int rect_rule = RECT_TIGHT;
  bool mark_depth_only = false;
  unsigned rowsum_wgs = 2048u;
  unsigned grad_fill_wgs = 512u;
  bool chain_sum_lanes = false;
};
RasterKnobs read_knobs();

struct BlendPlan {
  enum Fwd { FWD_TILE, FWD_WAVE } fwd;
  bool want_qmask;
  bool bwd_scan;
  uint32_t seg;
  bool seg_on, seg_reuse;
  uint32_t long_thr;
};
BlendPlan blend_plan(const RasterKnobs& k, int footprint_class, int64_t I, int num_tiles);

struct BwdState {
  uint32_t* cidx;
  float* rows;
  uint32_t *pair_off, *pair_owner;
  float* partials;
  float* tau_partials;
  char* temp;
  size_t temp_bytes, np_max, total;
};

GeomState carve_geom(void* blob, int P, int num_tiles);
int launch_tile_order(const uint32_t* work, int num_tiles, uint32_t* order, hipStream_t st, uint32_t* n_long = nullptr,
                      uint32_t long_thr = 0, uint32_t long_max = 0);
int occlusion_buckets(int num_tiles);
BinState carve_binning(void* blob, int64_t I, int num_tiles, uint32_t seg);
ImageState carve_image(void* blob, int W, int H);
BwdState carve_bwd(void* blob, int P, int64_t I);

constexpr int TS_THREADS = 256, TS_BLOCK = 4096;
size_t tile_sort_table_bytes(int64_t n);
template <typename KeyT>
int tile_sort(const KeyT* keys_in, int64_t n, int bits, KeyT* keys_tmp, uint32_t* vals_tmp, KeyT* keys_out,
              uint32_t* vals_out, uint32_t* table, hipStream_t st);
size_t tile_sort_library_bytes(int64_t n);
template <typename KeyT>
int tile_sort_library(const KeyT* keys_in, int64_t n, int bits, KeyT* keys_out, uint32_t* vals_out, void* temp,
                      size_t temp_bytes, hipStream_t st);

int launch_blend_fwd(int mode, const KParams& kp, const BlendPlan& plan, int P, int64_t I, const GeomState& gs,
                     const BinState& bs, const ImageState& im, float* out_color, float* out_normal, float* out_depth,
                     float* out_alpha, void* per_gaussian, hipStream_t st);

__device__ inline int lane_value(int v, int src) { return __builtin_amdgcn_readlane(v, src); }
__device__ inline uint32_t lane_value(uint32_t v, int src) { return (uint32_t)__builtin_amdgcn_readlane((int)v, src); }
__device__ inline float lane_value(float v, int src) {
  return __builtin_bit_cast(float, __builtin_amdgcn_readlane(__builtin_bit_cast(int, v), src));
}

__device__ inline int dealt_rank(int num_waves, int wave, int lane) {
  return lane < 16 ? lane * num_waves + wave : ((lane >> 4) * num_waves + wave) * 16 + (lane & 15);
}
__device__ inline int strided_rank(int P) {
  const int num_waves = (int)(gridDim.x * (blockDim.x >> 6));
  const int wave = (int)(blockIdx.x * (blockDim.x >> 6) + (threadIdx.x >> 6));
  const int r = dealt_rank(num_waves, wave, (int)(threadIdx.x & 63));
  return r < P ? r : -1;
}

constexpr int RB_LW = 4, RB_LS = 4;
__host__ __device__ inline uint32_t rank_bucket_log2(uint32_t x) { return 31u - (uint32_t)__builtin_clz(x); }
__host__ __device__ inline uint32_t rank_bucket(int r, int nb, uint32_t nvalid) {
  if (r < 0 || nvalid == 0u) return 0u;
  const uint32_t ur = (uint32_t)r, unb = (uint32_t)nb;
  if (ur >= nvalid) return unb - 1u;
  const uint32_t eq = (nvalid - 1u) / unb + 1u;
  uint32_t J = 0u;
  if ((eq >> RB_LW) != 0u) {
    J = rank_bucket_log2(eq >> RB_LW) + 2u;
    if (J > (unb >> (RB_LS + 1))) J = unb >> (RB_LS + 1);
  }
  const uint32_t front_ranks = J ? 1u << (RB_LW + RB_LS + J - 1u) : 0u, front_buckets = J << RB_LS;
  if (ur < front_ranks) {
    const uint32_t q = ur >> RB_LW;
    if ((q >> RB_LS) == 0u) return q;
    const uint32_t k = rank_bucket_log2(q) - RB_LS;
    return (k << RB_LS) + (q >> k);
  }
  const uint32_t b = front_buckets + (uint32_t)(((unsigned long long)(ur - front_ranks) * (unb - front_buckets)) /
                                                (unsigned long long)(nvalid - front_ranks));
  return b < unb ? b : unb - 1u;
}

typedef float f2 __attribute__((ext_vector_type(2)));
__device__ inline f2 f2s(float x) { return f2{x, x}; }
__device__ inline f2 fma2(f2 a, f2 b, f2 c) { return __builtin_elementwise_fma(a, b, c); }
__device__ inline f2 sel2(bool c0, bool c1, f2 a, f2 b) { return f2{c0 ? a.x : b.x, c1 ? a.y : b.y}; }

typedef unsigned long long lmask;
struct cmask {
  unsigned long long bits;
};
enum { LM_OGT = 2, LM_OGE = 3, LM_OLT = 4, LM_OLE = 5 };
__device__ inline cmask mask_lt(float a, float b) { return cmask{__builtin_amdgcn_fcmpf(a, b, LM_OLT)}; }
__device__ inline cmask mask_le(float a, float b) { return cmask{__builtin_amdgcn_fcmpf(a, b, LM_OLE)}; }
__device__ inline cmask mask_gt(float a, float b) { return cmask{__builtin_amdgcn_fcmpf(a, b, LM_OGT)}; }
__device__ inline cmask mask_ge(float a, float b) { return cmask{__builtin_amdgcn_fcmpf(a, b, LM_OGE)}; }
__device__ inline lmask operator&(cmask a, cmask b) { return a.bits & b.bits; }
__device__ inline lmask operator&(lmask a, cmask b) { return a & b.bits; }
__device__ inline lmask operator&(cmask a, lmask b) { return a.bits & b; }
__device__ inline lmask operator|(cmask a, cmask b) { return a.bits | b.bits; }
__device__ inline lmask operator~(cmask a) { return ~a.bits; }
__device__ inline int mask_count(lmask m) { return __builtin_popcountll(m); }
__device__ inline float mask_sel(lmask m, float a, float b) {
  float r;
  asm("v_cndmask_b32_e64 %0, %1, %2, %3" : "=v"(r) : "v"(b), "v"(a), "s"(m));
  return r;
}
__device__ inline uint32_t mask_sel(lmask m, uint32_t a, uint32_t b) {
  uint32_t r;
  asm("v_cndmask_b32_e64 %0, %1, %2, %3" : "=v"(r) : "v"(b), "v"(a), "s"(m));
  return r;
}
__device__ inline float mask_sel0(lmask m, float a) {
  float r;
  asm("v_cndmask_b32_e64 %0, 0, %1, %2" : "=v"(r) : "v"(a), "s"(m));
  return r;
}
__device__ inline uint32_t mask_one(lmask m) {
  uint32_t r;
  asm("v_cndmask_b32_e64 %0, 0, 1, %1" : "=v"(r) : "s"(m));
  return r;
}
__device__ inline f2 mask_sel2(lmask m0, lmask m1, f2 a, f2 b) { return f2{mask_sel(m0, a.x, b.x), mask_sel(m1, a.y, b.y)}; }
__device__ inline f2 mask_sel2_0(lmask m0, lmask m1, f2 a) { return f2{mask_sel0(m0, a.x), mask_sel0(m1, a.y)}; }

template <int CTRL>
__device__ inline float dpp_mov(float v) {
  return __builtin_bit_cast(
      float, __builtin_amdgcn_update_dpp(0, __builtin_bit_cast(int, v), CTRL, 0xf, 0xf, false));
}

template <int K>
__device__ inline float sel4(const float (&t)[4], bool m0, bool m1) {
  const float lo = m0 ? t[(1 + K) & 3] : t[K & 3];
  const float hi = m0 ? t[(3 + K) & 3] : t[(2 + K) & 3];
  return m1 ? hi : lo;
}

__device__ inline float wave_reduce16(const float (&v)[16], int lane) {
  const bool b0 = lane & 1, b1 = lane & 2;
  float u[8];
#pragma unroll
  for (int k = 0; k < 8; ++k) {
    const float send = b0 ? v[k] : v[k + 8];
    const float keep = b0 ? v[k + 8] : v[k];
    u[k] = keep + dpp_mov<0xb1>(send);
  }
  float t[4];
#pragma unroll
  for (int k = 0; k < 4; ++k) {
    const float send = b1 ? u[k] : u[k + 4];
    const float keep = b1 ? u[k + 4] : u[k];
    t[k] = keep + dpp_mov<0x4e>(send);
  }
  const bool m0 = lane & 4, m1 = lane & 8;
  float r = sel4<0>(t, m0, m1);
  r += dpp_mov<0x124>(sel4<1>(t, m0, m1));
  r += dpp_mov<0x128>(sel4<2>(t, m0, m1));
  r += dpp_mov<0x12c>(sel4<3>(t, m0, m1));
  {
    float a = r, b = r;
    asm volatile("s_nop 1\n\tv_permlane16_swap_b32 %0, %1" : "+v"(a), "+v"(b));
    r = a + b;
    a = r; b = r;
    asm volatile("s_nop 1\n\tv_permlane32_swap_b32 %0, %1" : "+v"(a), "+v"(b));
    r = a + b;
  }
  return r;
}

__host__ __device__ constexpr int red16_slot(int pos) {
  constexpr int m[16] = {G_MX, G_MY, G_CONX, G_NX, G_CONY, G_CONZ, G_ZLO, G_NY, G_OPAC, G_R, G_G, G_NZ, G_B, G_PZ, G_ZHI, G_Q};
  return m[pos];
}
__device__ inline int red16_lane_slot(int lane) {
  const int pos = 4 * (lane >> 4) + 2 * (lane & 1) + ((lane >> 1) & 1);
  constexpr unsigned long long packed = [] {
    unsigned long long w = 0;
    for (int q = 0; q < 16; ++q) w |= (unsigned long long)red16_slot(q) << (4 * q);
    return w;
  }();
  return (int)((packed >> (4 * pos)) & 15ull);
}

#define PINGS_SWAP3(op, a0, b0, a1, b1, a2, b2)                                     \
  asm volatile("s_nop 1\n\t" op " %0, %3\n\t" op " %1, %4\n\t" op " %2, %5"         \
               : "+v"(a0), "+v"(a1), "+v"(a2), "+v"(b0), "+v"(b1), "+v"(b2))
#define PINGS_SWAP4(op, a0, b0, a1, b1, a2, b2, a3, b3)                             \
  asm volatile("s_nop 1\n\t" op " %0, %4\n\t" op " %1, %5\n\t" op " %2, %6\n\t" op " %3, %7" \
               : "+v"(a0), "+v"(a1), "+v"(a2), "+v"(a3), "+v"(b0), "+v"(b1), "+v"(b2), "+v"(b3))
#define PINGS_SWAP5(op, a0, b0, a1, b1, a2, b2, a3, b3, a4, b4)                     \
  asm volatile("s_nop 1\n\t" op " %0, %5\n\t" op " %1, %6\n\t" op " %2, %7\n\t" op " %3, %8\n\t" op " %4, %9" \
               : "+v"(a0), "+v"(a1), "+v"(a2), "+v"(a3), "+v"(a4), "+v"(b0), "+v"(b1), "+v"(b2), "+v"(b3), "+v"(b4))
#define PINGS_SWAP8(op, a0, b0, a1, b1, a2, b2, a3, b3, a4, b4, a5, b5, a6, b6, a7, b7)                        \
  asm volatile("s_nop 1\n\t" op " %0, %8\n\t" op " %1, %9\n\t" op " %2, %10\n\t" op " %3, %11\n\t"             \
               op " %4, %12\n\t" op " %5, %13\n\t" op " %6, %14\n\t" op " %7, %15"                             \
               : "+v"(a0), "+v"(a1), "+v"(a2), "+v"(a3), "+v"(a4), "+v"(a5), "+v"(a6), "+v"(a7),               \
                 "+v"(b0), "+v"(b1), "+v"(b2), "+v"(b3), "+v"(b4), "+v"(b5), "+v"(b6), "+v"(b7))

__device__ inline void pair_add(float& r0, float& r1, float a0, float a1, float b0, float b1) {
  const f2 r = f2{a0, a1} + f2{b0, b1};
  r0 = r.x;
  r1 = r.y;
}

template <bool ZERO6>
__device__ inline float wave_reduce16_swap(const f2 (&v2)[16], int lane) {
  float s[16];
#pragma unroll
  for (int q = 0; q < 16; ++q) {
    const bool zero = ZERO6 && ((q & 3) == 3 || (q & 7) == 6);
    s[q] = zero ? 0.f : v2[red16_slot(q)].x + v2[red16_slot(q)].y;
  }
  float u[8], t[4];
  if (ZERO6) {
    PINGS_SWAP5("v_permlane32_swap_b32", s[0], s[8], s[1], s[9], s[2], s[10], s[4], s[12], s[5], s[13]);
    pair_add(u[0], u[1], s[0], s[1], s[8], s[9]);
    pair_add(u[4], u[5], s[4], s[5], s[12], s[13]);
    u[2] = s[2] + s[10];
    float z = 0.f;
    PINGS_SWAP3("v_permlane16_swap_b32", u[0], u[4], u[1], u[5], u[2], z);
    pair_add(t[0], t[1], u[0], u[1], u[4], u[5]);
    t[2] = u[2] + z;
    t[3] = 0.f;
  } else {
    PINGS_SWAP8("v_permlane32_swap_b32", s[0], s[8], s[1], s[9], s[2], s[10], s[3], s[11], s[4], s[12], s[5], s[13],
                s[6], s[14], s[7], s[15]);
#pragma unroll
    for (int k = 0; k < 8; k += 2) pair_add(u[k], u[k + 1], s[k], s[k + 1], s[k + 8], s[k + 9]);
    PINGS_SWAP4("v_permlane16_swap_b32", u[0], u[4], u[1], u[5], u[2], u[6], u[3], u[7]);
#pragma unroll
    for (int k = 0; k < 4; k += 2) pair_add(t[k], t[k + 1], u[k], u[k + 1], u[k + 4], u[k + 5]);
  }
  const bool b0 = lane & 1, b1 = lane & 2;
  float x[2];
#pragma unroll
  for (int k = 0; k < 2; ++k) {
    const float send = b0 ? t[k] : t[k + 2];
    const float keep = b0 ? t[k + 2] : t[k];
    x[k] = keep + dpp_mov<0xb1>(send);
  }
  float r = (b1 ? x[1] : x[0]) + dpp_mov<0x4e>(b1 ? x[0] : x[1]);
  r += dpp_mov<0x124>(r);
  r += dpp_mov<0x128>(r);
  asm volatile("" : "+v"(r));
  return r;
}

__device__ inline float wave_reduce_sum_dpp(float v) {
  v += __builtin_bit_cast(float, __builtin_amdgcn_update_dpp(0, __builtin_bit_cast(int, v), 0xb1, 0xf, 0xf, false));
  v += __builtin_bit_cast(float, __builtin_amdgcn_update_dpp(0, __builtin_bit_cast(int, v), 0x4e, 0xf, 0xf, false));
  v += __builtin_bit_cast(float, __builtin_amdgcn_update_dpp(0, __builtin_bit_cast(int, v), 0x124, 0xf, 0xf, false));
  v += __builtin_bit_cast(float, __builtin_amdgcn_update_dpp(0, __builtin_bit_cast(int, v), 0x128, 0xf, 0xf, false));
  v += __builtin_bit_cast(float, __builtin_amdgcn_update_dpp(0, __builtin_bit_cast(int, v), 0x142, 0xa, 0xf, false));
  v += __builtin_bit_cast(float, __builtin_amdgcn_update_dpp(0, __builtin_bit_cast(int, v), 0x143, 0xc, 0xf, false));
  return v;
}

__device__ inline uint32_t wave_reduce_sum_u32_dpp(uint32_t v) {
  v += (uint32_t)__builtin_amdgcn_update_dpp(0, (int)v, 0xb1, 0xf, 0xf, false);
  v += (uint32_t)__builtin_amdgcn_update_dpp(0, (int)v, 0x4e, 0xf, 0xf, false);
  v += (uint32_t)__builtin_amdgcn_update_dpp(0, (int)v, 0x124, 0xf, 0xf, false);
  v += (uint32_t)__builtin_amdgcn_update_dpp(0, (int)v, 0x128, 0xf, 0xf, false);
  v += (uint32_t)__builtin_amdgcn_update_dpp(0, (int)v, 0x142, 0xa, 0xf, false);
  v += (uint32_t)__builtin_amdgcn_update_dpp(0, (int)v, 0x143, 0xc, 0xf, false);
  return v;
}

__device__ inline float wave_sum_to_all(float v) {
  v = wave_reduce_sum_dpp(v);
  return __builtin_bit_cast(float, __builtin_amdgcn_readlane(__builtin_bit_cast(int, v), 63));
}

__device__ inline uint32_t wave_inclusive_sum(uint32_t v, int lane) {
#pragma unroll
  for (int d = 1; d < 64; d <<= 1) {
    const uint32_t u = __shfl_up(v, d, 64);
    if (lane >= d) v += u;
  }
  return v;
}

__device__ inline uint32_t wave_inclusive_sum_dpp(uint32_t v) {
  v += (uint32_t)__builtin_amdgcn_update_dpp(0, (int)v, 0x111, 0xf, 0xf, false);
  v += (uint32_t)__builtin_amdgcn_update_dpp(0, (int)v, 0x112, 0xf, 0xf, false);
  v += (uint32_t)__builtin_amdgcn_update_dpp(0, (int)v, 0x114, 0xf, 0xf, false);
  v += (uint32_t)__builtin_amdgcn_update_dpp(0, (int)v, 0x118, 0xf, 0xf, false);
  v += (uint32_t)__builtin_amdgcn_update_dpp(0, (int)v, 0x142, 0xa, 0xf, false);
  v += (uint32_t)__builtin_amdgcn_update_dpp(0, (int)v, 0x143, 0xc, 0xf, false);
  return v;
}

template <bool FROM_RANGES>
__device__ inline void tile_order_body(const uint32_t* __restrict__ work_in, const uint2* __restrict__ ranges,
                                       int num_tiles, uint32_t* __restrict__ order, uint32_t* __restrict__ n_long,
                                       uint32_t long_thr, uint32_t long_max) {
  __shared__ uint32_t hist[1024];
  __shared__ uint32_t base[1024];
  __shared__ uint32_t wtot[16];
  const int tid = threadIdx.x, lane = tid & 63, wave = tid >> 6;
  auto work = [&](int t) -> uint32_t {
    if constexpr (FROM_RANGES) { const uint2 r = ranges[t]; return r.y - r.x; }
    else return work_in[t];
  };
  hist[tid] = 0u;
  __syncthreads();
  for (int t = tid; t < num_tiles; t += 1024) atomicAdd(&hist[min(work(t) >> 4, 1023u)], 1u);
  __syncthreads();
  const uint32_t v = hist[1023 - tid];
  uint32_t incl = wave_inclusive_sum(v, lane);
  if (lane == 63) wtot[wave] = incl;
  __syncthreads();
#pragma unroll
  for (int w = 0; w < 16; ++w) incl += w < wave ? wtot[w] : 0u;
  base[tid] = incl;
  hist[1023 - tid] = incl - v;
  __syncthreads();
  for (int t = tid; t < num_tiles; t += 1024) order[atomicAdd(&hist[min(work(t) >> 4, 1023u)], 1u)] = (uint32_t)t;
  if (n_long) {
    const uint32_t bin = long_thr >> 4;
    if (bin > 1023u) {
      if (tid == 0) *n_long = 0u;
    } else {
      const uint32_t kmax = 1023u - bin;
      const uint32_t k = (uint32_t)tid;
      if (k <= kmax && base[k] <= long_max && (k == kmax || base[k + 1] > long_max)) *n_long = base[k];
      if (tid == 0 && base[0] > long_max) *n_long = 0u;
    }
  }
}

struct LiveOp {
  __host__ __device__ uint32_t operator()(const float& w) const { return w > 0.f ? 1u : 0u; }
};
struct PopOp {
  __host__ __device__ uint32_t operator()(const uint8_t& m) const { return (uint32_t)__builtin_popcount((unsigned)m & 15u); }
};
struct RowRanges {
  int P;
  const uint32_t *offsets_sorted, *tiles_sorted, *cidx;
  __host__ __device__ uint32_t row_begin(uint32_t r) const { return cidx[offsets_sorted[r] - tiles_sorted[r]]; }
  __host__ __device__ uint32_t row_end(uint32_t r) const { return cidx[offsets_sorted[r]]; }
  __host__ __device__ uint32_t operator()(const uint32_t& r) const {
    if (r >= (uint32_t)P) return 0u;
    return (row_end(r) - row_begin(r) + (uint32_t)CH - 1u) / (uint32_t)CH;
  }
};

constexpr int SCAN_THREADS = 1024, SCAN_BLOCK = 4 * SCAN_THREADS;
constexpr int64_t SCAN_MAX = (int64_t)SCAN_BLOCK * SCAN_BLOCK;
size_t raster_scan_bytes(int64_t n);
int raster_scan_u32(const uint32_t* in, int64_t n, bool inclusive, uint32_t* out, void* temp, size_t temp_bytes,
                    bool library, hipStream_t st);
struct TileOrderJob {
  const uint32_t* work = nullptr;
  int num_tiles = 0;
  uint32_t *order = nullptr, *n_long = nullptr;
  uint32_t long_thr = 0, long_max = 0;
};
int raster_scan_live(const float* inst_w, int64_t n, uint32_t* cidx, void* temp, size_t temp_bytes, bool library,
                     const TileOrderJob& job, hipStream_t st);
int raster_scan_pop(const uint8_t* inst_qmask, int64_t n, uint32_t* cidx, void* temp, size_t temp_bytes, bool library,
                    const TileOrderJob& job, hipStream_t st);
int raster_scan_chunks(const RowRanges& rr, uint32_t* pair_off, uint32_t* pair_owner, void* temp, size_t temp_bytes,
                       bool library, hipStream_t st);

__device__ inline float edge_min_q(float a, float b, float c, float d_fixed, float lo, float hi) {
  const float t = fminf(fmaxf(-(b * d_fixed) * __builtin_amdgcn_rcpf(c), lo), hi);
  const float q0 = a * d_fixed * d_fixed, q1 = 2.f * b * d_fixed * t, q2 = c * t * t;
  return (q0 + q1 + q2) - 2e-5f * (q0 + fabsf(q1) + q2);
}

__device__ inline bool footprint_misses_rect(float mx, float my, float cx, float cy, float cz, float thr,
                                             float x0, float x1, float y0, float y1) {
  if (mx >= x0 && mx <= x1 && my >= y0 && my <= y1) return false;
  const float lx = x0 - mx, hx = x1 - mx, ly = y0 - my, hy = y1 - my;
  float m = edge_min_q(cx, cy, cz, lx, ly, hy);
  m = fminf(m, edge_min_q(cx, cy, cz, hx, ly, hy));
  m = fminf(m, edge_min_q(cz, cy, cx, ly, lx, hx));
  m = fminf(m, edge_min_q(cz, cy, cx, hy, lx, hx));
  return m > thr;
}

__device__ inline uint32_t quadrant_mask(float mx, float my, float opacity, float cx, float cy, float cz,
                                         float X0, float Y0) {
  const float thr = 2.f * __logf(255.f * opacity) + 2e-3f;
  uint32_t m = 0;
#pragma unroll
  for (int q = 0; q < 4; ++q) {
    const float x0 = X0 + (float)(8 * (q & 1)), y0 = Y0 + (float)(8 * (q >> 1));
    if (!footprint_misses_rect(mx, my, cx, cy, cz, thr, x0, x0 + 7.f, y0, y0 + 7.f)) m |= 1u << q;
  }
  return m;
}

}
}
```

### pings_amd/csrc/raster_fwd.hip

```cpp
#include <hipcub/hipcub.hpp>

#include <algorithm>
#include <chrono>
#include <type_traits>

#include "raster_common.hpp"

namespace pings {
namespace raster {

__device__ inline void to_camera(const float* __restrict__ V, float x, float y, float z, float& px,
                                 float& py, float& pz) {
  px = ((V[0] * x + V[4] * y) + V[8] * z) + V[12];
  py = ((V[1] * x + V[5] * y) + V[9] * z) + V[13];
  pz = ((V[2] * x + V[6] * y) + V[10] * z) + V[14];
}

__global__ __launch_bounds__(256) void mark_visible_kernel(const float* __restrict__ pos, int N,
                                                            const float* __restrict__ V,
                                                            const float* __restrict__ Pm,
                                                            uint8_t* __restrict__ present, int depth_only) {
  const int i = blockIdx.x * blockDim.x + threadIdx.x;
  if (i >= N) return;
  float px, py, pz;
// ... 188 lines not shown
    for (int o = 32; o > 0; o >>= 1) tot += (uint32_t)__shfl_xor((int)tot, o, 64);
    if ((threadIdx.x & 63) == 0 && tot) {
      const int shard = stat_shard();
      atomicAdd(stats + STAT_PAIRS + shard, (unsigned long long)tot);
      atomicAdd(stats + STAT_VISIBLE + shard, (unsigned long long)__popcll(vis));
    }
  }
  if (!ds_head) return;
  uint32_t mx = key != CULLED_KEY ? key : 0u, mn = key != CULLED_KEY ? ~key : 0u;
#pragma unroll
  for (int o = 32; o > 0; o >>= 1) {
    mx = max(mx, (uint32_t)__shfl_xor((int)mx, o, 64));
    mn = max(mn, (uint32_t)__shfl_xor((int)mn, o, 64));
  }
  const int wave = threadIdx.x >> 6;
  if ((threadIdx.x & 63) == 0) { sm[wave] = mx; sm[4 + wave] = mn; }
  __syncthreads();
  if (threadIdx.x == 0) {
    mx = max(max(sm[0], sm[1]), max(sm[2], sm[3]));
    mn = max(max(sm[4], sm[5]), max(sm[6], sm[7]));
    if (mx | mn) {
      atomicMax(&ds_head[blockIdx.x % DS_SHARDS], mx);
      atomicMax(&ds_head[DS_SHARDS + blockIdx.x % DS_SHARDS], mn);
    }
  }
}

constexpr int SMALL_RECT = 8;

struct RectLane {
  uint32_t g, n;
  int xmin, ymin, wdt, hgt;
};
template <typename Serial, typename CoopBegin, typename Coop>
__device__ inline void walk_rects(const RectLane& me, int gx, Serial serial, CoopBegin coop_begin, Coop coop) {
  const int lane = threadIdx.x & 63;
  if (me.n != 0u && me.n <= (uint32_t)SMALL_RECT) {
    int x = 0, y = 0;
    for (uint32_t k = 0; k < me.n; ++k) {
      serial(me.xmin + x, me.ymin + y);
      if (++x == me.wdt) { x = 0; ++y; }
    }
  }
  unsigned long long m = __ballot(me.n > (uint32_t)SMALL_RECT);
  while (m) {
    const int src = __ffsll((long long)m) - 1;
    m &= m - 1;
    const uint32_t n = lane_value(me.n, src);
    const int x0 = lane_value(me.xmin, src), y0 = lane_value(me.ymin, src), wdt = lane_value(me.wdt, src);
    const float inv_w = 1.0f / (float)wdt;
    coop_begin(src);
    for (uint32_t k0 = 0; k0 < n; k0 += 64) {
      const uint32_t k = k0 + (uint32_t)lane;
      const bool act = k < n;
      int yy = (int)((float)k * inv_w);
      int xx = (int)k - yy * wdt;
      if (xx < 0) { --yy; xx += wdt; }
      if (xx >= wdt) { ++yy; xx -= wdt; }
      coop(src, act ? x0 + xx : 0, act ? y0 + yy : 0, act);
    }
  }
}

__device__ inline RectLane rect_lane(int r, const uint32_t* __restrict__ gidx_sorted, const uint4* __restrict__ rect,
                                     uint32_t nvalid) {
  RectLane me{0u, 0u, 0, 0, 1, 1};
  if (r >= 0 && (uint32_t)r < nvalid) {
    me.g = gidx_sorted[r];
    const uint4 rc = rect[me.g];
    me.n = rc.w;
    me.xmin = (int)(rc.y & 0xFFFF);
    me.ymin = (int)(rc.y >> 16);
    me.wdt = max((int)(rc.z & 0xFFFF) - me.xmin, 1);
    me.hgt = max((int)(rc.z >> 16) - me.ymin, 1);
  }
  return me;
}

constexpr int SMALL_ITEMS = 16;
constexpr uint32_t SMALL_KEPT = 16u;

__device__ inline unsigned long long kept_bits(const unsigned long long* __restrict__ m, int s, int w) {
  const int i = s >> 6, sh = s & 63;
  const unsigned long long lo = m[i], hi = m[i + 1];
  const unsigned long long v = sh ? (lo >> sh) | (hi << (64 - sh)) : lo;
  return v & (~0ull >> (64 - w));
}

struct RowItems {
  int s0, gx, wdt, cpr;
  float inv_cpr;
  __device__ RowItems(int xmin, int ymin, int wdt_, int gx_)
      : s0(ymin * gx_ + xmin), gx(gx_), wdt(wdt_), cpr((wdt_ + 63) >> 6), inv_cpr(1.0f / (float)((wdt_ + 63) >> 6)) {}
  __device__ void at(uint32_t k, int& s, int& w) const {
    int y = (int)k, c = 0;
    if (cpr > 1) {
      y = (int)((float)k * inv_cpr);
      c = (int)k - y * cpr;
      if (c < 0) { --y; c += cpr; }
      if (c >= cpr) { ++y; c -= cpr; }
    }
    s = s0 + y * gx + 64 * c;
    w = min(64, wdt - 64 * c);
  }
};

__device__ inline uint32_t rect_items(const RectLane& me) {
  return me.n != 0u ? (uint32_t)(me.hgt * ((me.wdt + 63) >> 6)) : 0u;
}

template <typename Serial>
__device__ inline void walk_items_serial(const RectLane& me, uint32_t items, int gx,
                                         const unsigned long long* __restrict__ mrow, Serial serial) {
  const RowItems ri(me.xmin, me.ymin, me.wdt, gx);
  for (uint32_t k0 = 0; k0 < items; k0 += 4) {
    int s[4];
    unsigned long long b[4];
#pragma unroll
    for (int u = 0; u < 4; ++u) {
      int w;
      ri.at(min(k0 + (uint32_t)u, items - 1u), s[u], w);
      b[u] = kept_bits(mrow, s[u], w);
    }
#pragma unroll
    for (int u = 0; u < 4; ++u)
      if (k0 + (uint32_t)u < items) serial(s[u], b[u]);
  }
}

template <typename Begin, typename Step>
__device__ inline void walk_items_coop(unsigned long long big, const RectLane& me, uint32_t items, int gx, uint32_t bk,
                                       const unsigned long long* __restrict__ mask, int words, Begin begin, Step step) {
  const int lane = threadIdx.x & 63;
  while (big) {
    const int src = __ffsll((long long)big) - 1;
    big &= big - 1;
    const uint32_t n = lane_value(items, src);
    const RowItems ri(lane_value(me.xmin, src), lane_value(me.ymin, src), lane_value(me.wdt, src), gx);
    const unsigned long long* mrow = mask + (size_t)lane_value(bk, src) * words;
    begin(src);
    for (uint32_t k0 = 0; k0 < n; k0 += 64) {
      const uint32_t k = k0 + (uint32_t)lane;
      int sk = 0, w = 1;
      unsigned long long bits = 0ull;
      if (k < n) {
        ri.at(k, sk, w);
        bits = kept_bits(mrow, sk, w);
      }
      step(sk, bits);
    }
  }
}

__device__ inline float tile_min_alpha(float mx, float my, float o, float cx, float cy, float cz, float X0, float Y0) {
  const float x1 = X0 + 15.f, y1 = Y0 + 15.f;
  if (mx >= X0 && mx <= x1 && my >= Y0 && my <= y1) return 0.f;
  float qmax = 0.f;
#pragma unroll
  for (int c = 0; c < 4; ++c) {
    const float dx = ((c & 1) ? x1 : X0) - mx, dy = ((c & 2) ? y1 : Y0) - my;
    const float q0 = cx * dx * dx, q1 = 2.f * cy * dx * dy, q2 = cz * dy * dy;
    qmax = fmaxf(qmax, (q0 + q1 + q2) + 2e-5f * (q0 + fabsf(q1) + q2));
  }
  const float a = fminf(ALPHA_MAX, o * __expf(-0.5f * (qmax + 1e-3f)) * (1.f - 1e-5f));
  if (!(a >= ALPHA_MIN * 1.001f)) return 0.f;
  const float lx = X0 - mx, hx = x1 - mx, ly = Y0 - my, hy = y1 - my;
  float m = edge_min_q(cx, cy, cz, lx, ly, hy);
  m = fminf(m, edge_min_q(cx, cy, cz, hx, ly, hy));
  m = fminf(m, edge_min_q(cz, cy, cx, ly, lx, hx));
  m = fminf(m, edge_min_q(cz, cy, cx, hy, lx, hx));
  if (!(m > 1e-6f)) return 0.f;
  return a;
}

struct DsRange { uint32_t kmin, shift; };

__device__ inline DsRange ds_range(const uint32_t* __restrict__ head) { return DsRange{head[DS_KMIN], head[DS_SHIFT]}; }

__device__ inline DsRange ds_range_from_shards(const uint32_t* __restrict__ head, uint32_t (&sr)[2]) {
  if (threadIdx.x < 64) {
    uint32_t mx = head[threadIdx.x], mn = head[DS_SHARDS + threadIdx.x];
#pragma unroll
    for (int o = 32; o > 0; o >>= 1) {
      mx = max(mx, (uint32_t)__shfl_xor((int)mx, o, 64));
      mn = max(mn, (uint32_t)__shfl_xor((int)mn, o, 64));
    }
    if (threadIdx.x == 0) {
      const uint32_t kmin = ~mn;
      uint32_t shift = 0u;
      if (mx > kmin)
        while (((mx - kmin) >> shift) >= (uint32_t)DS_NB) ++shift;
      sr[0] = kmin;
      sr[1] = shift;
    }
  }
  __syncthreads();
  return DsRange{sr[0], sr[1]};
}

__global__ __launch_bounds__(256) void ds_hist_kernel(int P, const uint32_t* __restrict__ key, uint32_t* __restrict__ head,
                                                       uint32_t* __restrict__ cnt, uint32_t* __restrict__ pos) {
  __shared__ uint32_t sc[4];
  __shared__ uint32_t sr[2];
  const int g = blockIdx.x * 256 + threadIdx.x;
  const int lane = threadIdx.x & 63;
  const uint32_t k = g < P ? key[g] : 0u;
  const bool culled = g < P && k == CULLED_KEY;
  const bool active = g < P && !culled;
  const DsRange r = ds_range_from_shards(head, sr);
  if (blockIdx.x == 0 && threadIdx.x == 0) { head[DS_KMIN] = r.kmin; head[DS_SHIFT] = r.shift; }
  const uint32_t b = active ? (k - r.kmin) >> r.shift : 0xFFFFFFFFu;
  unsigned long long todo = __ballot(active);
  const unsigned long long below = (1ull << lane) - 1ull;
  int my_leader = lane;
  uint32_t my_rank = 0u, group = 0u;
  while (todo) {
    const int leader = __ffsll((long long)todo) - 1;
    const uint32_t lb = (uint32_t)__builtin_amdgcn_readlane((int)b, leader);
    const unsigned long long m = __ballot(b == lb) & todo;
    if (b == lb) {
      my_leader = leader;
      my_rank = (uint32_t)__popcll(m & below);
      group = (uint32_t)__popcll(m);
    }
    todo &= ~m;
  }
  uint32_t base = 0u;
  if (active && my_leader == lane) base = atomicAdd(&cnt[b], group);
  base = (uint32_t)__shfl((int)base, my_leader, 64);
  if (active) pos[g] = base + my_rank;
  const unsigned long long bal = __ballot(culled);
  if (lane == 0) sc[threadIdx.x >> 6] = (uint32_t)__popcll(bal);
  __syncthreads();
  if (threadIdx.x == 0) cnt[DS_NB + blockIdx.x] = (sc[0] + sc[1]) + (sc[2] + sc[3]);
}

__global__ __launch_bounds__(256) void ds_scatter_kernel(int P, const uint32_t* __restrict__ key, const uint32_t* __restrict__ head,
                                                          const uint32_t* __restrict__ off, const uint32_t* __restrict__ pos,
                                                          uint32_t* __restrict__ tmp_key, uint32_t* __restrict__ tmp_idx,
                                                          uint32_t* __restrict__ gidx_sorted) {
  __shared__ uint32_t sc[4];
  const int g = blockIdx.x * 256 + threadIdx.x;
  const int lane = threadIdx.x & 63, wave = threadIdx.x >> 6;
  const uint32_t k = g < P ? key[g] : 0u;
  const bool culled = g < P && k == CULLED_KEY;
  if (g < P && !culled) {
    const DsRange r = ds_range(head);
    const uint32_t b = (k - r.kmin) >> r.shift;
    const uint32_t slot = off[b] + pos[g];
    tmp_key[slot] = k;
    tmp_idx[slot] = (uint32_t)g;
  }
  const unsigned long long bal = __ballot(culled);
  if (lane == 0) sc[wave] = (uint32_t)__popcll(bal);
  __syncthreads();
  if (culled) {
    uint32_t before = (uint32_t)__popcll(bal & ((1ull << lane) - 1ull));
    for (int w = 0; w < wave; ++w) before += sc[w];
    gidx_sorted[off[DS_NB + blockIdx.x] + before] = (uint32_t)g;
  }
}

__global__ __launch_bounds__(256) void ds_rank_kernel(const uint32_t* __restrict__ tmp_key, const uint32_t* __restrict__ tmp_idx,
                                                       uint32_t* __restrict__ head, const uint32_t* __restrict__ off,
                                                       uint32_t* __restrict__ gidx_sorted, uint32_t* __restrict__ rank_of,
                                                       uint32_t* __restrict__ nvalid) {
  const uint32_t n = off[DS_NB];
  const uint32_t s = blockIdx.x * 256u + threadIdx.x;
  if (s == 0u) *nvalid = n;
  if (s >= n) return;
  const uint32_t k = tmp_key[s], id = tmp_idx[s];
  const DsRange r = ds_range(head);
  const uint32_t b = (k - r.kmin) >> r.shift;
  const uint32_t lo = off[b], hi = off[b + 1];
  if (hi - lo > DS_LIMIT) {
    gidx_sorted[s] = id;
    rank_of[id] = s;
    if (s == lo) head[DS_FLAG] = 1u;
    return;
  }
  uint32_t rank = 0u;
  uint32_t t = lo;
  for (; t + 8u <= hi; t += 8u) {
    uint32_t kt[8], it[8];
#pragma unroll
    for (int u = 0; u < 8; ++u) { kt[u] = tmp_key[t + u]; it[u] = tmp_idx[t + u]; }
#pragma unroll
    for (int u = 0; u < 8; ++u) rank += (kt[u] < k || (kt[u] == k && it[u] < id)) ? 1u : 0u;
  }
  for (; t < hi; ++t) {
    const uint32_t kt = tmp_key[t], it = tmp_idx[t];
    rank += (kt < k || (kt == k && it < id)) ? 1u : 0u;
  }
  gidx_sorted[lo + rank] = id;
  rank_of[id] = lo + rank;
}

__global__ __launch_bounds__(256) void invert_perm_kernel(int P, const uint32_t* __restrict__ gidx_sorted,
                                                           uint32_t* __restrict__ rank_of) {
  const int r = blockIdx.x * 256 + threadIdx.x;
  if (r < P) rank_of[gidx_sorted[r]] = (uint32_t)r;
}

__global__ __launch_bounds__(64) void count_valid_kernel(int P, const uint32_t* __restrict__ depth_key_sorted,
                                                         uint32_t* __restrict__ nvalid) {
  const int lane = threadIdx.x;
  long long lo = 0, hi = P;
  while (lo < hi) {
    const long long span = hi - lo;
    const long long step = (span + 63) / 64;
    const long long pos = lo + (long long)lane * step;
    const bool valid = pos < hi && depth_key_sorted[pos] < CULLED_KEY;
    const int nv = __popcll(__ballot(valid));
    if (nv == 0) { hi = lo; break; }
    const long long last_valid = lo + (long long)(nv - 1) * step;
    lo = last_valid + 1;
    hi = min(hi, last_valid + step);
  }
  if (lane == 0) *nvalid = (uint32_t)lo;
}


template <bool DENSE>
__global__ __launch_bounds__(256) void occl_budget_kernel(int P, int gx, int nb,
                                                          const uint32_t* __restrict__ gidx_sorted,
                                                          const uint4* __restrict__ rect,
// ... 169 lines not shown
#pragma unroll
  for (int off = 32; off > 0; off >>= 1) kept_w += (uint32_t)__shfl_xor((int)kept_w, off, 64);
  if (lane == 0 && kept_w) atomicAdd(stats + STAT_KEPT + stat_shard(), (unsigned long long)kept_w);
}

template <typename KeyT>
__global__ __launch_bounds__(256) void duplicate_kernel(int P, int gx, int nb, int words,
                                                         const uint32_t* __restrict__ gidx_sorted,
                                                         const uint32_t* __restrict__ offsets_sorted,
                                                         const uint32_t* __restrict__ tiles_sorted,
                                                         const uint4* __restrict__ rect,
                                                         const unsigned long long* __restrict__ mask,
                                                         const uint32_t* __restrict__ nvalid,
                                                         KeyT* __restrict__ tile_key,
                                                         uint32_t* __restrict__ gval,
                                                         uint32_t* __restrict__ per_gaussian) {
  const int i = blockIdx.x * blockDim.x + threadIdx.x;
  if (i < P) per_gaussian[i] = 0u;
  const int r = strided_rank(P);
  const int lane = threadIdx.x & 63;
  const uint32_t kept = r >= 0 ? tiles_sorted[r] : 0u;
  const uint32_t nv = *nvalid;
  const RectLane me = rect_lane(kept != 0u ? r : -1, gidx_sorted, rect, nv);
  const uint32_t bk = kept != 0u ? rank_bucket(r, nb, nv) : 0u;
  uint32_t o = kept != 0u ? offsets_sorted[r] - kept : 0u;
  const uint32_t items = rect_items(me);
  const bool coop = items > (uint32_t)SMALL_ITEMS || kept > SMALL_KEPT;
  if (items != 0u && !coop)
    walk_items_serial(me, items, gx, mask + (size_t)bk * words, [&](int s, unsigned long long bits) {
      while (bits) {
        tile_key[o] = (KeyT)(s + __builtin_ctzll(bits));
        gval[o] = me.g;
        ++o;
        bits &= bits - 1;
      }
    });
  uint32_t so = 0, sg = 0;
  walk_items_coop(
      __ballot(items != 0u && coop), me, items, gx, bk, mask, words,
      [&](int src) {
        so = lane_value(o, src);
        sg = lane_value(me.g, src);
      },
      [&](int s, unsigned long long bits) {
        unsigned long long todo = __ballot(bits != 0ull);
        while (todo) {
          const int j = __ffsll((long long)todo) - 1;
          todo &= todo - 1;
          const uint32_t blo = lane_value((uint32_t)bits, j), bhi = lane_value((uint32_t)(bits >> 32), j);
          const int sj = lane_value(s, j);
          if (((lane < 32 ? blo : bhi) >> (lane & 31)) & 1u) {
            const uint32_t pos = so + __builtin_amdgcn_mbcnt_hi(bhi, __builtin_amdgcn_mbcnt_lo(blo, 0u));
            tile_key[pos] = (KeyT)(sj + lane);
            gval[pos] = sg;
          }
          so += (uint32_t)(__popc(blo) + __popc(bhi));
        }
      });
}

template <bool FROM_RANGES>
__global__ __launch_bounds__(1024) void tile_order_kernel(const uint32_t* __restrict__ work_in,
                                                          const uint2* __restrict__ ranges, int num_tiles,
                                                          uint32_t* __restrict__ order, uint32_t* __restrict__ n_long,
                                                          uint32_t long_thr, uint32_t long_max) {
  tile_order_body<FROM_RANGES>(work_in, ranges, num_tiles, order, n_long, long_thr, long_max);
}

int launch_tile_order(const uint32_t* work, int num_tiles, uint32_t* order, hipStream_t st, uint32_t* n_long,
                      uint32_t long_thr, uint32_t long_max) {
  hipLaunchKernelGGL(tile_order_kernel<false>, dim3(1), dim3(1024), 0, st, work, (const uint2*)nullptr, num_tiles, order,
                     n_long, long_thr, long_max);
  PINGS_LAUNCH_CHECK();
  return PINGS_OK;
}

template <typename KeyT>
__global__ __launch_bounds__(256) void tile_ranges_kernel(int64_t I, const KeyT* __restrict__ key,
                                                           uint2* __restrict__ ranges) {
  const int64_t i = (int64_t)blockIdx.x * blockDim.x + threadIdx.x;
  if (i >= I) return;
  const uint32_t t = (uint32_t)key[i];
  if (i == 0 || key[i - 1] != t) ranges[t].x = (uint32_t)i;
  if (i == I - 1 || key[i + 1] != t) ranges[t].y = (uint32_t)(i + 1);
}

struct AuxPtrs {
  const int32_t* p[8];
};
__global__ __launch_bounds__(64) void frame_summary_kernel(const uint32_t* __restrict__ overflow,
                                                           const unsigned long long* __restrict__ shards, AuxPtrs aux,
                                                           int aux_words, FrameSummary* __restrict__ out, uint32_t seq) {
  __shared__ unsigned long long part[3][64];
  const int lane = threadIdx.x;
  unsigned long long a0 = 0, a1 = 0, a2 = 0;
  for (int i = lane; i < STAT_SHARDS; i += 64) {
    a0 += shards[STAT_PAIRS + i]; a1 += shards[STAT_VISIBLE + i]; a2 += shards[STAT_KEPT + i];
  }
  part[0][lane] = a0; part[1][lane] = a1; part[2][lane] = a2;
  __syncthreads();
  if (lane < 3) {
    unsigned long long t = 0;
    for (int i = 0; i < 64; ++i) t += part[lane][i];
    out->stats[lane] = t;
  }
  if (lane == 4) out->overflow = overflow ? *overflow : 0u;
  if (lane >= 8 && lane < 16) out->aux[lane - 8] = (lane - 8 < aux_words && aux.p[lane - 8]) ? *aux.p[lane - 8] : 0;
  __threadfence_system();
  __syncthreads();
  if (lane == 0) __hip_atomic_store(&out->seq, seq, __ATOMIC_RELEASE, __HIP_MEMORY_SCOPE_SYSTEM);
}

static int make_params(const pings_raster_settings* s, int P, const RasterKnobs& knobs, KParams& kp) {
  if (int e = fill_camera(s, P, kp)) return e;
  kp.occ_amin = knobs.occ_amin;
  kp.rect_rule = knobs.rect_rule;
  kp.live = nullptr;
  kp.dyn_rows = 0;
  return PINGS_OK;
}

static int tile_bits(int num_tiles) {
  int b = 1;
  while ((1 << b) < num_tiles) ++b;
  return b;
}

}
}

using namespace pings::raster;

PINGS_API int pings_raster_mark_visible(const float* positions, int N,
                                        const pings_raster_settings* s, uint8_t* present,
                                        void* stream) {
  PINGS_ARG_CHECK(s && s->viewmatrix && s->projmatrix_raw, "null settings / matrices");
  if (N == 0) return PINGS_OK;
  PINGS_ARG_CHECK(N > 0 && positions && present, "null pointer");
  const int depth_only = read_knobs().mark_depth_only;
  hipLaunchKernelGGL(mark_visible_kernel, dim3(pings::ceil_div(N, 256)), dim3(256), 0,
                     pings::as_stream(stream), positions, N, s->viewmatrix, s->projmatrix_raw,
                     present, depth_only);
  PINGS_LAUNCH_CHECK();
  return PINGS_OK;
}

PINGS_API int pings_raster_rank_bucket(const int32_t* ranks, int64_t n, int occ_nb, uint32_t nvalid,
                                       uint32_t* buckets) {
  PINGS_ARG_CHECK(n >= 0 && occ_nb > 0 && (n == 0 || (ranks && buckets)), "null pointer / non-positive bucket count");
  for (int64_t i = 0; i < n; ++i) buckets[i] = rank_bucket(ranks[i], occ_nb, nvalid);
  return PINGS_OK;
}

PINGS_API int pings_raster_preprocess(const pings_raster_settings* s, int P, const float* means3D,
                                      const float* colors, const float* opacities,
                                      const float* scales, const float* rotations,
                                      void* geom_blob, int32_t* radii, int64_t* num_instances,
                                      int32_t* footprint_class, void* stream) {
  return pings_raster_preprocess_dyn(s, P, means3D, colors, opacities, scales, rotations, geom_blob, radii, nullptr, 0,
                                     nullptr, 0, nullptr, num_instances, footprint_class, stream);
}

PINGS_API int pings_raster_preprocess_dyn(const pings_raster_settings* s, int P, const float* means3D,
                                          const float* colors, const float* opacities, const float* scales,
                                          const float* rotations, void* geom_blob, int32_t* radii,
                                          const int32_t* live_rows_dev, int dyn_rows,
                                          const int32_t* const* aux_dev, int aux_words, int32_t* aux_host,
                                          int64_t* num_instances, int32_t* footprint_class, void* stream) {
  const RasterKnobs knobs = read_knobs();
  KParams kp;
  if (int e = make_params(s, P, knobs, kp)) return e;
  PINGS_ARG_CHECK(num_instances != nullptr && footprint_class != nullptr, "null output");
  *num_instances = 0;
  *footprint_class = 1;
  PINGS_ARG_CHECK(aux_words >= 0 && aux_words <= 8 && (aux_words == 0 || (aux_dev && aux_host)), "0..8 aux words");
  PINGS_ARG_CHECK(!live_rows_dev || (dyn_rows >= 0 && dyn_rows <= P), "dyn_rows must lie in 0..P");
  PINGS_ARG_CHECK(P > 0 || aux_words == 0, "aux words need a non-empty frame");
  if (P == 0) return PINGS_OK;
  kp.live = live_rows_dev;
  kp.dyn_rows = live_rows_dev ? dyn_rows : 0;
  PINGS_ARG_CHECK(P > 0 && means3D && colors && opacities && scales && rotations && geom_blob && radii,
                  "null pointer");
  hipStream_t st = pings::as_stream(stream);
  const int num_tiles = kp.gx * kp.gy;
  GeomState gs = carve_geom(geom_blob, P, num_tiles);
  const dim3 grid(pings::ceil_div(P, 256)), block(256);
  const bool occlusion = knobs.occlusion;
  bool library_sort = knobs.library_sort;
  PINGS_HIP_CHECK(hipMemsetAsync(gs.zero_begin, 0, gs.zero_bytes, st));
  {
    pings::prof::Scope ps("preprocess", st);
    with_mode(s->mode, [&](auto m) {
      hipLaunchKernelGGL(preprocess_kernel<m()>, grid, block, 0, st, kp, means3D, colors,
                         opacities, scales, rotations, gs.rec, gs.rect, gs.depth_key, gs.gidx, radii,
                         library_sort ? (uint32_t*)nullptr : gs.ds_head, gs.stats);
    });
    PINGS_LAUNCH_CHECK();
  }
  static thread_local FrameSummary* host_sum = nullptr;
  static thread_local FrameSummary* host_sum_dev = nullptr;
  static thread_local uint32_t frame_seq = 0;
  if (!host_sum) {
    PINGS_HIP_CHECK(hipHostMalloc(reinterpret_cast<void**>(&host_sum), sizeof(FrameSummary), hipHostMallocMapped | hipHostMallocPortable));
    PINGS_HIP_CHECK(hipHostGetDevicePointer(reinterpret_cast<void**>(&host_sum_dev), host_sum, 0));
    host_sum->seq = 0;
  }
  AuxPtrs aux;
  for (int i = 0; i < 8; ++i) aux.p[i] = i < aux_words ? aux_dev[i] : nullptr;
  for (int attempt = 0;; ++attempt) {
    size_t tb = gs.temp_bytes;
    if (library_sort) {
      pings::prof::Scope ps("depth_sort", st);
      PINGS_HIP_CHECK(hipcub::DeviceRadixSort::SortPairs(gs.temp, tb, gs.depth_key, gs.depth_key_sorted,
                                                         gs.gidx, gs.gidx_sorted, P, 0, 32, st));
      hipLaunchKernelGGL(count_valid_kernel, dim3(1), dim3(64), 0, st, P, gs.depth_key_sorted, gs.nvalid);
      PINGS_LAUNCH_CHECK();
      hipLaunchKernelGGL(invert_perm_kernel, grid, block, 0, st, P, gs.gidx_sorted, gs.rank_of);
      PINGS_LAUNCH_CHECK();
    } else {
      pings::prof::Scope ps("depth_sort", st);
      hipLaunchKernelGGL(ds_hist_kernel, grid, block, 0, st, P, gs.depth_key, gs.ds_head, gs.ds_cnt, gs.rank_of);
      PINGS_LAUNCH_CHECK();
      if (int e = raster_scan_u32(gs.ds_cnt, DS_NB + (int64_t)grid.x + 1, false, gs.ds_off, gs.temp, gs.temp_bytes,
                                  knobs.library_scan, st))
        return e;
      hipLaunchKernelGGL(ds_scatter_kernel, grid, block, 0, st, P, gs.depth_key, gs.ds_head, gs.ds_off, gs.rank_of,
                         gs.depth_key_sorted, gs.ds_idx, gs.gidx_sorted);
      PINGS_LAUNCH_CHECK();
      hipLaunchKernelGGL(ds_rank_kernel, grid, block, 0, st, gs.depth_key_sorted, gs.ds_idx, gs.ds_head, gs.ds_off,
                         gs.gidx_sorted, gs.rank_of, gs.nvalid);
      PINGS_LAUNCH_CHECK();
    }
    if (occlusion) {
      {
        pings::prof::Scope ps("occl_setup", st);
        if (attempt > 0)
          PINGS_HIP_CHECK(hipMemsetAsync(gs.occ_bucket, 0, sizeof(uint32_t) * (size_t)num_tiles * gs.occ_nb, st));
      }
      {
        pings::prof::Scope ps("occl_budget", st);
        hipLaunchKernelGGL(knobs.occ_walk_lanes ? occl_budget_kernel<false> : occl_budget_kernel<true>, grid, block, 0,
                           st, P, kp.gx, gs.occ_nb, gs.gidx_sorted, gs.rect, gs.rec, gs.nvalid, num_tiles, gs.occ_bucket);
        PINGS_LAUNCH_CHECK();
      }
    }
    {
      pings::prof::Scope ps("occl_scan", st);
      if (attempt > 0)
        PINGS_HIP_CHECK(hipMemsetAsync(gs.stats + STAT_KEPT, 0, STAT_RETRY_WORDS * sizeof(unsigned long long), st));
      hipLaunchKernelGGL(occl_scan_kernel, dim3(gs.occ_words), dim3(512), 0, st, num_tiles, gs.occ_nb, gs.occ_bucket,
                         gs.occ_bsat, gs.occ_mask, gs.occ_bmax);
      PINGS_LAUNCH_CHECK();
    }
    {
      pings::prof::Scope ps("tile_count_scan", st);
      hipLaunchKernelGGL(count_kept_kernel, grid, block, 0, st, P, kp.gx, gs.occ_nb, gs.occ_words, gs.gidx_sorted,
                         gs.rect, gs.occ_mask, gs.nvalid, gs.occ_bmax, gs.tiles_sorted, gs.stats);
      PINGS_LAUNCH_CHECK();
    }
    const uint32_t seq = ++frame_seq ? frame_seq : ++frame_seq;
    hipLaunchKernelGGL(frame_summary_kernel, dim3(1), dim3(64), 0, st,
                       library_sort ? (const uint32_t*)nullptr : gs.ds_head + DS_FLAG, gs.stats, aux, aux_words,
                       host_sum_dev, seq);
    PINGS_LAUNCH_CHECK();
    {
      pings::prof::Scope ps("tile_count_scan", st);
      if (int e = raster_scan_u32(gs.tiles_sorted, P, true, gs.offsets_sorted, gs.temp, gs.temp_bytes, knobs.library_scan, st))
        return e;
    }
    {
      const auto t_start = std::chrono::steady_clock::now();
      unsigned spins = 0;
      while (__atomic_load_n(&host_sum->seq, __ATOMIC_ACQUIRE) != seq) {
        if ((++spins & 0x3FFu) == 0) {
          const hipError_t q = hipStreamQuery(st);
          if (q == hipErrorNotReady) (void)hipGetLastError();
          else if (q != hipSuccess) PINGS_HIP_CHECK(q);
          if (std::chrono::steady_clock::now() - t_start > std::chrono::seconds(20)) {
            PINGS_HIP_CHECK(hipStreamSynchronize(st));
            PINGS_ARG_CHECK(__atomic_load_n(&host_sum->seq, __ATOMIC_ACQUIRE) == seq, "frame summary never arrived");
          }
        }
        __builtin_ia32_pause();
      }
    }
    if (host_sum->overflow == 0) break;
    library_sort = true;
  }
  const unsigned long long stats[3] = {host_sum->stats[0], host_sum->stats[1], host_sum->stats[2]};
  for (int i = 0; i < aux_words; ++i) aux_host[i] = host_sum->aux[i];
  PINGS_ARG_CHECK(stats[2] < 0x7FFFFFFFull, "more than 2^31 - 1 (Gaussian, tile) instances in this frame");
  *num_instances = (int64_t)stats[2];
  *footprint_class = (stats[1] > 0 && stats[0] > 16ull * stats[1]) ? 2 : 1;
  return PINGS_OK;
}

PINGS_API int pings_raster_render(const pings_raster_settings* s, int P, int64_t I,
                                  void* geom_blob, void* binning_blob, void* image_blob,
                                  float* out_color, float* out_normal,
                                  float* out_depth, float* out_alpha, void* per_gaussian,
                                  int footprint_class, void* stream) {
  const RasterKnobs knobs = read_knobs();
  KParams kp;
  if (int e = make_params(s, P, knobs, kp)) return e;
  PINGS_ARG_CHECK(out_color && out_depth && out_alpha && image_blob && binning_blob, "null pointer");
  PINGS_ARG_CHECK(s->mode == PINGS_RASTER_3DGS || out_normal, "surfel mode needs out_normal");
// ... 60 lines not shown
```

### pings_amd/csrc/raster_layout.hip

```cpp
#include <hipcub/hipcub.hpp>

#include <algorithm>
#include <cmath>
#include <cstdlib>
#include <cstring>

#include "raster_common.hpp"

namespace pings {
namespace raster {

static size_t sort_temp_bytes(int64_t n) {
  size_t a = 0, b = 0;
  (void)hipcub::DeviceRadixSort::SortPairs(nullptr, a, (uint32_t*)nullptr, (uint32_t*)nullptr,
                                     (uint32_t*)nullptr, (uint32_t*)nullptr, (int)n, 0, 32);
  (void)hipcub::DeviceScan::InclusiveSum(nullptr, b, (uint32_t*)nullptr, (uint32_t*)nullptr,
                                         (int)std::max<int64_t>(n, DS_NB + n / 256 + 2));
  size_t c = 0;
  (void)hipcub::DeviceRadixSort::SortPairs(nullptr, c, (uint16_t*)nullptr, (uint16_t*)nullptr,
                                           (uint32_t*)nullptr, (uint32_t*)nullptr, (int)n, 0, 16);
  if (c > a) a = c;
  a = std::max(a, std::max(tile_sort_library_bytes(n), tile_sort_table_bytes(n)));
  a = std::max(a, raster_scan_bytes(std::max<int64_t>(n, DS_NB + n / 256 + 2)));
  return align_up(a > b ? a : b) + 256;
}

int occlusion_buckets(int num_tiles) {
  int nb = 256;
  while (nb > 32 && (size_t)nb * (size_t)num_tiles > ((size_t)1 << 21)) nb >>= 1;
  return nb;
}

GeomState carve_geom(void* blob, int P, int num_tiles) {
  Carver c(blob);
  GeomState g;
  const size_t n = (size_t)(P > 0 ? P : 1);
  const size_t nt = (size_t)(num_tiles > 0 ? num_tiles : 1);
  g.rec = c.take<float4>(4 * n);
  g.rect = c.take<uint4>(n);
  g.depth_key = c.take<uint32_t>(n);
  g.depth_key_sorted = c.take<uint32_t>(n);
  g.gidx = c.take<uint32_t>(n);
  g.gidx_sorted = c.take<uint32_t>(n);
  g.rank_of = c.take<uint32_t>(n);
  g.tiles_sorted = c.take<uint32_t>(n);
  g.offsets_sorted = c.take<uint32_t>(n);
  g.occ_nb = occlusion_buckets((int)nt);
  g.occ_bucket = c.take<uint32_t>(nt * (size_t)g.occ_nb);
  g.stats = c.take<unsigned long long>(STAT_WORDS);
  g.occ_bmax = g.stats ? reinterpret_cast<uint32_t*>(g.stats + STAT_BMAX) : nullptr;
  const size_t nblk = (n + 255) / 256;
  g.ds_words = DS_HEAD + (size_t)DS_NB + nblk;
  g.ds_head = c.take<uint32_t>(g.ds_words);
  g.ds_cnt = g.ds_head ? g.ds_head + DS_HEAD : nullptr;
  g.zero_begin = reinterpret_cast<char*>(g.occ_bucket);
  g.zero_bytes = g.ds_head ? align_up((size_t)(reinterpret_cast<char*>(g.ds_head + g.ds_words) - g.zero_begin)) : 0;
  g.occ_bsat = c.take<uint16_t>(nt);
  g.occ_words = (int)((nt + 63) / 64);
  g.occ_mask = c.take<unsigned long long>((size_t)g.occ_nb * (size_t)g.occ_words + 1);
  g.nvalid = c.take<uint32_t>(1);
  g.ds_off = c.take<uint32_t>((size_t)DS_NB + nblk + 1);
  g.ds_idx = c.take<uint32_t>(n);
  g.summary = c.take<FrameSummary>(1);
  g.temp_bytes = sort_temp_bytes((int64_t)n);
  g.temp = c.take<char>(g.temp_bytes);
  g.total = c.total();
  return g;
}

BinState carve_binning(void* blob, int64_t I, int num_tiles, uint32_t seg) {
  Carver c(blob);
  BinState b;
  const size_t n = (size_t)(I > 0 ? I : 1);
  b.point_list = c.take<uint32_t>(n);
  b.ranges = c.take<uint2>((size_t)num_tiles);
  b.inst_w = c.take<float>(n + 1);
  b.inst_qmask = c.take<uint8_t>(n + 1);
  b.inst_cnt = c.take<uint32_t>(n);
  b.inst_wq = c.take<float>(4 * n);
  b.inst_cntq = c.take<uint32_t>(4 * n);
  b.tile_key = c.take<uint32_t>(n);
  b.tile_key_sorted = c.take<uint32_t>(n);
  b.gval = c.take<uint32_t>(n);
  b.slot_val = c.take<uint32_t>(n);
  b.tile_order = c.take<uint32_t>(2 * (size_t)num_tiles + 4);
  b.tile_work = c.take<uint32_t>((size_t)num_tiles);
  b.tile_maxc = c.take<uint32_t>((size_t)num_tiles);
  const size_t sg = (size_t)seg;
  b.seg_max_units = sg ? (uint32_t)(n / sg + n / (2 * sg) + 64) : 1u;
  if (b.seg_max_units > (1u << 20)) b.seg_max_units = 1u << 20;
  b.seg_head = c.take<uint32_t>(4);
  b.seg_unit_tile = c.take<uint32_t>(b.seg_max_units);
  b.seg_unit_seg = c.take<uint32_t>(b.seg_max_units);
  b.seg_tile_unit0 = c.take<uint32_t>((size_t)num_tiles);
  b.seg_P = c.take<float>((size_t)b.seg_max_units * 256);
  b.seg_slab = c.take<float>((size_t)b.seg_max_units * 256 * 10);
  const bool reuse = sg > 0 && sg <= 65535;
  b.seg_rel = c.take<uint16_t>(reuse ? (size_t)b.seg_max_units * 4 * sg : 1);
  b.seg_nrel = c.take<uint32_t>((size_t)b.seg_max_units * 4);
  b.temp_bytes = sort_temp_bytes((int64_t)n);
  b.temp = c.take<char>(b.temp_bytes);
  b.total = c.total();
  return b;
}

ImageState carve_image(void* blob, int W, int H) {
  Carver c(blob);
  ImageState im;
  im.final_T = c.take<float>((size_t)W * H);
  im.n_contrib = c.take<uint32_t>((size_t)W * H);
  im.total = c.total();
  return im;
}

BwdState carve_bwd(void* blob, int P, int64_t I) {
  Carver c(blob);
  BwdState b;
  const size_t ni = (size_t)(I > 0 ? I : 1), n = 4 * ni, np = (size_t)(P > 0 ? P : 1);
  b.np_max = n / CH + np + 1;
  b.cidx = c.take<uint32_t>(ni + 2);
  b.pair_off = c.take<uint32_t>(np + 1);
  b.pair_owner = c.take<uint32_t>(b.np_max);
  b.partials = c.take<float>(b.np_max * GRAD_ROW);
  b.tau_partials = c.take<float>(ceil_div<size_t>(std::max(np, b.np_max), 256) * 6);
  b.temp_bytes = std::max(raster_scan_bytes((int64_t)ni + 1), raster_scan_bytes((int64_t)np + 1));
  b.temp = c.take<char>(b.temp_bytes);
  b.rows = c.take<float>(n * GRAD_ROW);
  b.total = c.total();
  return b;
}

RasterKnobs read_knobs() {
  RasterKnobs k;
  if (const char* e = getenv("PINGS_BLEND_PPL")) k.blend_ppl = atoi(e);
  if (const char* e = getenv("PINGS_BLEND_BWD")) k.blend_bwd = strcmp(e, "pixel") != 0 ? RasterKnobs::BWD_SCAN : RasterKnobs::BWD_PIXEL;
  if (const char* e = getenv("PINGS_BLEND_SEG")) k.blend_seg = (uint32_t)atoi(e);
  if (const char* e = getenv("PINGS_BLEND_SEG_REUSE")) k.seg_reuse = atoi(e) != 0;
  if (const char* e = getenv("PINGS_BWD_LONG")) {
    const long v = atol(e);
    k.bwd_long = v <= 0 ? 0xFFFFFFF0u : (uint32_t)((v + 15) / 16 * 16);
  }
  if (const char* e = getenv("PINGS_RASTER_OCCLUSION")) k.occlusion = atoi(e) != 0;
  if (const char* e = getenv("PINGS_DEPTH_SORT")) k.library_sort = e[0] == 'l';
  if (const char* e = getenv("PINGS_TILE_SORT")) k.library_tile_sort = e[0] == 'l';
  if (const char* e = getenv("PINGS_RASTER_SCAN")) k.library_scan = e[0] == 'l';
  if (const char* e = getenv("PINGS_OCC_AMIN")) k.occ_amin = fminf(fmaxf((float)atof(e), 1.0f / 255.0f), 0.99f);
  if (const char* e = getenv("PINGS_OCC_WALK")) k.occ_walk_lanes = e[0] == 'l';
  if (const char* e = getenv("PINGS_RASTER_RECT")) k.rect_rule = e[0] == '3' ? RECT_3SIGMA : e[0] == 'e' ? RECT_ELLIPSE : RECT_TIGHT;
  if (const char* e = getenv("PINGS_MARK_VISIBLE")) k.mark_depth_only = e[0] == 'd';
  if (const char* e = getenv("PINGS_ROWSUM_WGS")) k.rowsum_wgs = (unsigned)std::min(std::max(atoi(e), 1), 65535);
  if (const char* e = getenv("PINGS_GRAD_FILL")) k.grad_fill_wgs = e[0] == 'l' ? 0u : (unsigned)std::min(std::max(atoi(e), 1), 65535);
  if (const char* e = getenv("PINGS_CHAIN_SUM")) k.chain_sum_lanes = e[0] == 'l';
  return k;
}

BlendPlan blend_plan(const RasterKnobs& k, int footprint_class, int64_t I, int num_tiles) {
  BlendPlan p;
  p.bwd_scan = k.blend_bwd == RasterKnobs::BWD_AUTO ? footprint_class != 2 : k.blend_bwd == RasterKnobs::BWD_SCAN;
  p.want_qmask = p.bwd_scan;
  const bool tile_wave = k.blend_ppl == 4 || (k.blend_ppl == 0 && footprint_class == 2 && !p.want_qmask);
  p.fwd = tile_wave ? BlendPlan::FWD_TILE : BlendPlan::FWD_WAVE;
  p.seg = k.blend_seg;
  p.seg_on = p.seg > 0 && I > (int64_t)num_tiles * (p.seg / 4) && I > 2 * (int64_t)p.seg;
  p.seg_reuse = p.seg <= 65535u && k.seg_reuse;
  p.long_thr = k.bwd_long;
  return p;
}

}
}

using namespace pings::raster;

PINGS_API size_t pings_raster_geom_bytes(int P, int image_height, int image_width) {
  const int nt = pings::ceil_div(image_width, TILE) * pings::ceil_div(image_height, TILE);
  return carve_geom(nullptr, P, nt).total;
}

PINGS_API size_t pings_raster_binning_bytes(int64_t num_instances, int image_height,
                                            int image_width) {
  const int nt = pings::ceil_div(image_width, TILE) * pings::ceil_div(image_height, TILE);
  return carve_binning(nullptr, num_instances, nt, read_knobs().blend_seg).total;
}

PINGS_API size_t pings_raster_backward_bytes(int P, int64_t num_instances) {
  return carve_bwd(nullptr, P, num_instances).total;
}

PINGS_API size_t pings_raster_image_bytes(int image_height, int image_width) {
  return carve_image(nullptr, image_width, image_height).total;
}

__global__ void slots_to_ids_kernel(int64_t I, const uint32_t* __restrict__ list, const uint32_t* __restrict__ gval,
                                    uint32_t* __restrict__ out) {
  const int64_t i = (int64_t)blockIdx.x * blockDim.x + threadIdx.x;
  if (i < I) out[i] = gval[list[i]];
}


PINGS_API int pings_raster_debug_lists(const void* binning_blob, int64_t I, int image_height,
                                       int image_width, uint32_t* point_list, uint32_t* ranges_xy,
                                       void* stream) {
  PINGS_ARG_CHECK(binning_blob && ranges_xy, "null pointer");
  const int nt = pings::ceil_div(image_width, TILE) * pings::ceil_div(image_height, TILE);
  BinState bs = carve_binning(const_cast<void*>(binning_blob), I, nt, read_knobs().blend_seg);
  hipStream_t st = pings::as_stream(stream);
  if (I > 0 && point_list) {
    hipLaunchKernelGGL(slots_to_ids_kernel, dim3((unsigned)pings::ceil_div<int64_t>(I, 256)), dim3(256), 0, st, I,
                       bs.point_list, bs.gval, point_list);
    PINGS_LAUNCH_CHECK();
  }
  PINGS_HIP_CHECK(hipMemcpyAsync(ranges_xy, bs.ranges, sizeof(uint2) * (size_t)nt,
                                 hipMemcpyDeviceToDevice, st));
  return PINGS_OK;
}

PINGS_API int pings_raster_debug_occlusion(const void* geom_blob, int P, int image_height, int image_width,
                                           uint32_t* occ_bucket, uint16_t* occ_bsat, int32_t* occ_nb, void* stream) {
  PINGS_ARG_CHECK(occ_nb, "null pointer");
  const int nt = pings::ceil_div(image_width, TILE) * pings::ceil_div(image_height, TILE);
  *occ_nb = occlusion_buckets(nt);
  if (!occ_bucket && !occ_bsat) return PINGS_OK;
  PINGS_ARG_CHECK(geom_blob && occ_bucket && occ_bsat, "null pointer");
  GeomState gs = carve_geom(const_cast<void*>(geom_blob), P, nt);
  hipStream_t st = pings::as_stream(stream);
  PINGS_HIP_CHECK(hipMemcpyAsync(occ_bucket, gs.occ_bucket, sizeof(uint32_t) * (size_t)nt * (size_t)gs.occ_nb,
                                 hipMemcpyDeviceToDevice, st));
  PINGS_HIP_CHECK(hipMemcpyAsync(occ_bsat, gs.occ_bsat, sizeof(uint16_t) * (size_t)nt, hipMemcpyDeviceToDevice, st));
  return PINGS_OK;
}

PINGS_API int pings_raster_debug_image(const void* image_blob, int image_height, int image_width,
                                       float* final_T, uint32_t* n_contrib, void* stream) {
  PINGS_ARG_CHECK(image_blob && final_T && n_contrib, "null pointer");
  ImageState im = carve_image(const_cast<void*>(image_blob), image_width, image_height);
  hipStream_t st = pings::as_stream(stream);
  const size_t n = (size_t)image_height * image_width;
  PINGS_HIP_CHECK(hipMemcpyAsync(final_T, im.final_T, sizeof(float) * n, hipMemcpyDeviceToDevice, st));
  PINGS_HIP_CHECK(hipMemcpyAsync(n_contrib, im.n_contrib, sizeof(uint32_t) * n,
                                 hipMemcpyDeviceToDevice, st));
  return PINGS_OK;
}
```

Baseline: 2739 Mpix/s.

## Specialise backward blend for Gaussians provably interior to a tile

Adds a per-tile, per-Gaussian test that proves a surfel is fully inside the tile's alpha, ray-plane and depth-clamp bounds. For such interior Gaussians the backward blend loop uses a specialised path that drops alpha clamping, validity checks, depth clamp branches and three gradient accumulators, and a smaller wave reduction. It adds classification cost per loaded Gaussian and a second instantiation of the inner loop, which can raise register pressure. A host debug entry point exposes the classifier for testing.

```diff
diff --git a/include/pings_hip.h b/include/pings_hip.h
--- a/include/pings_hip.h
+++ b/include/pings_hip.h
@@ -117,6 +117,8 @@
                                            void* stream);
 PINGS_API int pings_raster_rank_bucket(const int32_t* ranks, int64_t n, int occ_nb, uint32_t nvalid,
                                        uint32_t* buckets);
+PINGS_API int pings_raster_debug_interior(const float* records, const float* tile_origins, int64_t n, float cxp,
+                                          float cyp, float fx, float fy, uint8_t* flags);
 
 
 PINGS_API size_t pings_raster2d_geom_bytes(int P, int image_height, int image_width);
diff --git a/pings_amd/_abi.py b/pings_amd/_abi.py
--- a/pings_amd/_abi.py
+++ b/pings_amd/_abi.py
@@ -209,6 +209,7 @@
     "pings_raster_debug_image": (i32, [vp, i32, i32, vp, vp, vp]),
     "pings_raster_debug_occlusion": (i32, [vp, i32, i32, i32, vp, vp, C.POINTER(C.c_int32), vp]),
     "pings_raster_rank_bucket": (i32, [vp, i64, i32, C.c_uint32, vp]),
+    "pings_raster_debug_interior": (i32, [vp, vp, i64, f32, f32, f32, f32, vp]),
     "pings_raster2d_geom_bytes": (sz, [i32, i32, i32]),
     "pings_raster2d_binning_bytes": (sz, [i64, i32, i32]),
     "pings_raster2d_image_bytes": (sz, [i32, i32]),
diff --git a/pings_amd/csrc/raster_bwd.hip b/pings_amd/csrc/raster_bwd.hip
--- a/pings_amd/csrc/raster_bwd.hip
+++ b/pings_amd/csrc/raster_bwd.hip
@@ -19,11 +19,12 @@
     const uint32_t* __restrict__ n_contrib, const float* __restrict__ out_depth, const float* __restrict__ dL_dcolor,
     const float* __restrict__ dL_dnormal, const float* __restrict__ dL_ddepth, const float* __restrict__ dL_dalpha,
     const float* __restrict__ inst_w, const uint32_t* __restrict__ cidx, float* __restrict__ rows,
-    const uint32_t* __restrict__ tile_order) {
+    const uint32_t* __restrict__ tile_order, int interior_on) {
   __shared__ float4 sA[BATCH], sB[BATCH], sC[BATCH], sD[BATCH];
   __shared__ uint32_t sRow[BATCH];
   __shared__ float4 sG[BATCH][4];
   __shared__ uint8_t sList[BATCH];
+  __shared__ uint8_t sInt[BATCH];
 
   const int lane = threadIdx.x;
   const int tile = (int)tile_order[blockIdx.x];
@@ -36,12 +37,14 @@
 
   f2 rx = {0.f, 0.f};
   float ry[2] = {0.f, 0.f};
+  TileRays rays = {0.f, 0.f, 0.f, 0.f};
   if (MODE == MODE_SURFEL) {
     const float cxp = (p.prcp ? p.prcp[0] : 0.5f) * (float)p.W - 0.5f;
     const float cyp = (p.prcp ? p.prcp[1] : 0.5f) * (float)p.H - 0.5f;
     rx = f2{(pixf_x.x - cxp) / p.fx, (pixf_x.y - cxp) / p.fx};
 #pragma unroll
     for (int r = 0; r < 2; ++r) ry[r] = (pixf_y[r] - cyp) / p.fy;
+    rays = tile_rays_uniform(tile_rays(tileX0, tileY0, cxp, cyp, p.fx, p.fy));
   }
 
   const uint2 range = ranges[tile];
@@ -112,11 +115,16 @@
       const float4 rb = rec[4 * (size_t)g + 1];
       sA[lane] = ra;
       sB[lane] = rb;
-      sC[lane] = rec[4 * (size_t)g + 2];
-      if (MODE == MODE_SURFEL) sD[lane] = rec[4 * (size_t)g + 3];
+      const float4 rc = rec[4 * (size_t)g + 2];
+      sC[lane] = rc;
+      float4 rd = make_float4(0.f, 0.f, 0.f, 0.f);
+      if (MODE == MODE_SURFEL) sD[lane] = rd = rec[4 * (size_t)g + 3];
       const bool live = inst_w[slot] > 0.f;
       sRow[lane] = live ? cidx[slot] : DEAD_ROW;
       if (live) hit = quadrant_mask(ra.x, ra.y, ra.z, rb.x, rb.y, rb.z, tileX0, tileY0) != 0u;
+      if (MODE == MODE_SURFEL)
+        sInt[lane] = hit && interior_on && blend_interior(ra.x, ra.y, ra.z, ra.w, rb.x, rb.y, rb.z, rb.w, rc.w, rd.x, rd.y,
+                                                          rd.z, tileX0, tileY0, rays) ? 1 : 0;
     }
     const unsigned long long bal = __ballot(hit);
     if (hit) sList[__builtin_amdgcn_mbcnt_hi((uint32_t)(bal >> 32), __builtin_amdgcn_mbcnt_lo((uint32_t)bal, 0u))] = (uint8_t)lane;
@@ -127,14 +135,17 @@
       for (int e = lane; e < BATCH * 4; e += 64) z[e] = zero;
     }
     __syncthreads();
+    unsigned long long int_bits = 0ull;
+    if (MODE == MODE_SURFEL) int_bits = __ballot(lane < cnt && sInt[sList[lane < cnt ? lane : 0] & (BATCH - 1)] != 0);
 
     int i0 = cnt > 0 ? (int)sList[cnt - 1] : 0;
     int i1 = cnt > 1 ? (int)sList[cnt - 2] : 0;
     float4 a0 = sA[i0], b0 = sB[i0], c0 = sC[i0], n0 = make_float4(0.f, 0.f, 0.f, 0.f);
     float4 a1, b1, c1, n1 = n0;
     if (MODE == MODE_SURFEL) n0 = sD[i0];
-    auto trip = [&](const float4& ca, const float4& cb, const float4& cc, const float4& cn, const int j)
+    auto trip = [&](auto interior_c, const float4& ca, const float4& cb, const float4& cc, const float4& cn, const int j)
                     __attribute__((always_inline)) {
+      constexpr bool INT = MODE == MODE_SURFEL && decltype(interior_c)::value;
       const uint32_t idx = (uint32_t)(start + j);
       const f2 dx = f2s(ca.x) - pixf_x;
       const f2 p0 = f2s(-0.5f) * ((f2s(cb.x) * dx) * dx);
@@ -150,9 +161,9 @@
         const f2 power = (p0 - f2s(0.5f * (cb.z * dy * dy))) - pxy * f2s(dy);
         Gs[r] = f2{__expf(power.x), __expf(power.y)};
         raw[r] = f2s(ca.z) * Gs[r];
-        alpha[r] = f2{fminf(ALPHA_MAX, raw[r].x), fminf(ALPHA_MAX, raw[r].y)};
-        valid[r][0] = idx < last[r][0] && (power.x <= 0.0f) && (alpha[r].x >= ALPHA_MIN);
-        valid[r][1] = idx < last[r][1] && (power.y <= 0.0f) && (alpha[r].y >= ALPHA_MIN);
+        alpha[r] = INT ? raw[r] : f2{fminf(ALPHA_MAX, raw[r].x), fminf(ALPHA_MAX, raw[r].y)};
+        valid[r][0] = idx < last[r][0] && (INT || ((power.x <= 0.0f) && (alpha[r].x >= ALPHA_MIN)));
+        valid[r][1] = idx < last[r][1] && (INT || ((power.y <= 0.0f) && (alpha[r].y >= ALPHA_MIN)));
         any_v = any_v || valid[r][0] || valid[r][1];
       }
       if (!__any(any_v)) return;
@@ -161,6 +172,7 @@
 #pragma clang fp contract(fast)
       f2 v2[16];
       if (MODE != MODE_SURFEL) v2[G_NX] = v2[G_NY] = v2[G_NZ] = v2[G_Q] = v2[G_ZLO] = v2[G_ZHI] = f2{0.f, 0.f};
+      if (INT) v2[G_ZLO] = v2[G_ZHI] = v2[G_PZ] = f2{0.f, 0.f};
       const float zlo = ca.w - cb.w, zhi = ca.w + cb.w;
       const float zlo_m = fminf(zlo, zhi);
       const f2 cxdx = f2s(cb.x) * dx;
@@ -180,20 +192,26 @@
         if (MODE == MODE_SURFEL) {
           sdot += (f2s(cn.x) * gN0[r] + f2s(cn.y) * gN1[r]) + f2s(cn.z) * gN2[r];
           const f2 den = fma2(f2s(cn.x), rx, f2s(fmaf(cn.y, ry[r], cn.z)));
-          const bool hit0 = den.x < -DEN_EPS, hit1 = den.y < -DEN_EPS;
           const f2 inv_den = {__builtin_amdgcn_rcpf(den.x), __builtin_amdgcn_rcpf(den.y)};
-          const f2 d0 = sel2(hit0, hit1, f2s(cc.w) * inv_den, f2s(ca.w));
-          const f2 d = {__builtin_amdgcn_fmed3f(d0.x, zlo_m, zhi), __builtin_amdgcn_fmed3f(d0.y, zlo_m, zhi)};
-          sdot = fma2(d, gD[r], sdot);
-          const f2 gd = gD[r] * w;
-          const bool lo0 = d0.x < zlo, lo1 = d0.y < zlo, hi0 = d0.x > zhi, hi1 = d0.y > zhi;
-          const bool mid0 = !lo0 && !hi0, mid1 = !lo1 && !hi1;
-          const f2 zero = {0.f, 0.f};
-          acc(G_ZLO, sel2(lo0, lo1, gd, zero));
-          acc(G_ZHI, sel2(hi0, hi1, gd, zero));
-          const f2 gq = sel2(mid0 && hit0, mid1 && hit1, gd * inv_den, zero);
+          f2 d0 = f2s(cc.w) * inv_den, gq;
+          if (INT) {
+            sdot = fma2(d0, gD[r], sdot);
+            gq = mul_rounded(gD[r] * w, inv_den);
+          } else {
+            const bool hit0 = den.x < -DEN_EPS, hit1 = den.y < -DEN_EPS;
+            d0 = sel2(hit0, hit1, d0, f2s(ca.w));
+            const f2 d = {__builtin_amdgcn_fmed3f(d0.x, zlo_m, zhi), __builtin_amdgcn_fmed3f(d0.y, zlo_m, zhi)};
+            sdot = fma2(d, gD[r], sdot);
+            const f2 gd = gD[r] * w;
+            const bool lo0 = d0.x < zlo, lo1 = d0.y < zlo, hi0 = d0.x > zhi, hi1 = d0.y > zhi;
+            const bool mid0 = !lo0 && !hi0, mid1 = !lo1 && !hi1;
+            const f2 zero = {0.f, 0.f};
+            acc(G_ZLO, sel2(lo0, lo1, gd, zero));
+            acc(G_ZHI, sel2(hi0, hi1, gd, zero));
+            gq = sel2(mid0 && hit0, mid1 && hit1, gd * inv_den, zero);
+            acc(G_PZ, sel2(mid0 && !hit0, mid1 && !hit1, gd, zero));
+          }
           acc(G_Q, gq);
-          acc(G_PZ, sel2(mid0 && !hit0, mid1 && !hit1, gd, zero));
           const f2 gden = -gq * d0;
           v2[G_NX] = fma2(gden, rx, first ? gN0[r] * w : fma2(gN0[r], w, v2[G_NX]));
           v2[G_NY] = fma2(gden, f2s(ry[r]), first ? gN1[r] * w : fma2(gN1[r], w, v2[G_NY]));
@@ -205,7 +223,8 @@
         f2 dLda = sdot - Bs[r];
         Bs[r] = fma2(av, dLda, Bs[r]);
         dLda = dLda * Tn;
-        dLda = sel2(valid[r][0] && raw[r].x <= ALPHA_MAX, valid[r][1] && raw[r].y <= ALPHA_MAX, dLda, f2{0.f, 0.f});
+        dLda = sel2(valid[r][0] && (INT || raw[r].x <= ALPHA_MAX), valid[r][1] && (INT || raw[r].y <= ALPHA_MAX), dLda,
+                    f2{0.f, 0.f});
         acc(G_OPAC, Gs[r] * dLda);
         const f2 dLp = raw[r] * dLda;
         const f2 qx = cxdx + f2s(cb.y * dyv[r]), qy = pxy + f2s(cb.z * dyv[r]);
@@ -217,7 +236,7 @@
         acc(G_CONZ, uy * qy);
         T[r] = Tn;
       }
-      const float tot = wave_reduce16_swap<MODE != MODE_SURFEL>(v2, lane) * red_scale;
+      const float tot = wave_reduce16_swap<MODE != MODE_SURFEL ? RED_ZERO6 : INT ? RED_ZERO3 : RED_FULL>(v2, lane) * red_scale;
       if (red_store) reinterpret_cast<float*>(&sG[j][0])[red_slot] = tot;
       }
     };
@@ -227,7 +246,8 @@
         a1 = sA[i1]; b1 = sB[i1]; c1 = sC[i1];
         if (MODE == MODE_SURFEL) n1 = sD[i1];
         i0 = (int)sList[jj > 1 ? jj - 2 : 0];
-        trip(a0, b0, c0, n0, j);
+        if ((int_bits >> jj) & 1ull) trip(std::true_type{}, a0, b0, c0, n0, j);
+        else trip(std::false_type{}, a0, b0, c0, n0, j);
       }
       if (jj == 0) break;
       {
@@ -235,7 +255,8 @@
         a0 = sA[i0]; b0 = sB[i0]; c0 = sC[i0];
         if (MODE == MODE_SURFEL) n0 = sD[i0];
         i1 = (int)sList[jj > 2 ? jj - 3 : 0];
-        trip(a1, b1, c1, n1, j);
+        if ((int_bits >> (jj - 1)) & 1ull) trip(std::true_type{}, a1, b1, c1, n1, j);
+        else trip(std::false_type{}, a1, b1, c1, n1, j);
       }
     }
     __syncthreads();
@@ -274,13 +295,13 @@
     const uint32_t* __restrict__ n_contrib, const float* __restrict__ out_depth, const float* __restrict__ dL_dcolor,
     const float* __restrict__ dL_dnormal, const float* __restrict__ dL_ddepth, const float* __restrict__ dL_dalpha,
     const float* __restrict__ inst_w, const uint32_t* __restrict__ cidx, float* __restrict__ rows,
-    const uint32_t* __restrict__ tile_order, uint32_t num_tiles, GradFill fill) {
+    const uint32_t* __restrict__ tile_order, uint32_t num_tiles, GradFill fill, int interior_on) {
   if (blockIdx.x >= num_tiles) {
     grad_fill_part(fill, blockIdx.x - num_tiles, gridDim.x - num_tiles);
     return;
   }
   blend_bwd_tile_body<MODE>(p, ranges, point_list, rec, gval, final_T, n_contrib, out_depth, dL_dcolor, dL_dnormal,
-                            dL_ddepth, dL_dalpha, inst_w, cidx, rows, tile_order);
+                            dL_ddepth, dL_dalpha, inst_w, cidx, rows, tile_order, interior_on);
 }
 
 __global__ __launch_bounds__(64) void tile_max_contrib_kernel(int W, int H, int gx, const uint32_t* __restrict__ n_contrib,
@@ -1102,7 +1123,7 @@
         hipLaunchKernelGGL((blend_bwd_tile_kernel<M>), dim3((unsigned)num_tiles + fill_wgs), dim3(64), 0, st, bp,
                            bs.ranges, bs.point_list, gs.rec, bs.gval, im.final_T, im.n_contrib, out_depth, dL_dcolor,
                            dL_dnormal, dL_ddepth, dL_dalpha, bs.inst_w, bw.cidx, bw.rows, order, (uint32_t)num_tiles,
-                           fill);
+                           fill, (int)plan.interior_bwd);
       }
     });
     PINGS_LAUNCH_CHECK();
diff --git a/pings_amd/csrc/raster_common.hpp b/pings_amd/csrc/raster_common.hpp
--- a/pings_amd/csrc/raster_common.hpp
+++ b/pings_amd/csrc/raster_common.hpp
@@ -1,4 +1,5 @@
 #pragma once
+#include <cmath>
 #include <cstdlib>
 #include <type_traits>
 
@@ -175,6 +176,7 @@
   unsigned rowsum_wgs = 2048u;
   unsigned grad_fill_wgs = 512u;
   bool chain_sum_lanes = false;
+  bool blend_interior = true;
 };
 RasterKnobs read_knobs();
 
@@ -185,6 +187,7 @@
   uint32_t seg;
   bool seg_on, seg_reuse;
   uint32_t long_thr;
+  bool interior_bwd;
 };
 BlendPlan blend_plan(const RasterKnobs& k, int footprint_class, int64_t I, int num_tiles);
 
@@ -263,6 +266,10 @@
 typedef float f2 __attribute__((ext_vector_type(2)));
 __device__ inline f2 f2s(float x) { return f2{x, x}; }
 __device__ inline f2 fma2(f2 a, f2 b, f2 c) { return __builtin_elementwise_fma(a, b, c); }
+__device__ inline f2 mul_rounded(f2 a, f2 b) {
+#pragma clang fp contract(off)
+  return a * b;
+}
 __device__ inline f2 sel2(bool c0, bool c1, f2 a, f2 b) { return f2{c0 ? a.x : b.x, c1 ? a.y : b.y}; }
 
 typedef unsigned long long lmask;
@@ -371,6 +378,11 @@
 #define PINGS_SWAP5(op, a0, b0, a1, b1, a2, b2, a3, b3, a4, b4)                     \
   asm volatile("s_nop 1\n\t" op " %0, %5\n\t" op " %1, %6\n\t" op " %2, %7\n\t" op " %3, %8\n\t" op " %4, %9" \
                : "+v"(a0), "+v"(a1), "+v"(a2), "+v"(a3), "+v"(a4), "+v"(b0), "+v"(b1), "+v"(b2), "+v"(b3), "+v"(b4))
+#define PINGS_SWAP7(op, a0, b0, a1, b1, a2, b2, a3, b3, a4, b4, a5, b5, a6, b6)                                \
+  asm volatile("s_nop 1\n\t" op " %0, %7\n\t" op " %1, %8\n\t" op " %2, %9\n\t" op " %3, %10\n\t"              \
+               op " %4, %11\n\t" op " %5, %12\n\t" op " %6, %13"                                               \
+               : "+v"(a0), "+v"(a1), "+v"(a2), "+v"(a3), "+v"(a4), "+v"(a5), "+v"(a6),                          \
+                 "+v"(b0), "+v"(b1), "+v"(b2), "+v"(b3), "+v"(b4), "+v"(b5), "+v"(b6))
 #define PINGS_SWAP8(op, a0, b0, a1, b1, a2, b2, a3, b3, a4, b4, a5, b5, a6, b6, a7, b7)                        \
   asm volatile("s_nop 1\n\t" op " %0, %8\n\t" op " %1, %9\n\t" op " %2, %10\n\t" op " %3, %11\n\t"             \
                op " %4, %12\n\t" op " %5, %13\n\t" op " %6, %14\n\t" op " %7, %15"                             \
@@ -383,12 +395,14 @@
   r1 = r.y;
 }
 
-template <bool ZERO6>
+enum { RED_FULL = 0, RED_ZERO6 = 1, RED_ZERO3 = 2 };
+template <int ZEROS>
 __device__ inline float wave_reduce16_swap(const f2 (&v2)[16], int lane) {
+  constexpr bool ZERO6 = ZEROS == RED_ZERO6, ZERO3 = ZEROS == RED_ZERO3;
   float s[16];
 #pragma unroll
   for (int q = 0; q < 16; ++q) {
-    const bool zero = ZERO6 && ((q & 3) == 3 || (q & 7) == 6);
+    const bool zero = (ZERO6 && ((q & 3) == 3 || (q & 7) == 6)) || (ZERO3 && (q == 6 || q == 13 || q == 14));
     s[q] = zero ? 0.f : v2[red16_slot(q)].x + v2[red16_slot(q)].y;
   }
   float u[8], t[4];
@@ -402,6 +416,17 @@
     pair_add(t[0], t[1], u[0], u[1], u[4], u[5]);
     t[2] = u[2] + z;
     t[3] = 0.f;
+  } else if (ZERO3) {
+    PINGS_SWAP7("v_permlane32_swap_b32", s[0], s[8], s[1], s[9], s[2], s[10], s[3], s[11], s[4], s[12], s[5], s[13],
+                s[7], s[15]);
+    pair_add(u[0], u[1], s[0], s[1], s[8], s[9]);
+    pair_add(u[2], u[3], s[2], s[3], s[10], s[11]);
+    pair_add(u[4], u[5], s[4], s[5], s[12], s[13]);
+    u[7] = s[7] + s[15];
+    u[6] = 0.f;
+    PINGS_SWAP4("v_permlane16_swap_b32", u[0], u[4], u[1], u[5], u[2], u[6], u[3], u[7]);
+#pragma unroll
+    for (int k = 0; k < 4; k += 2) pair_add(t[k], t[k + 1], u[k], u[k + 1], u[k + 4], u[k + 5]);
   } else {
     PINGS_SWAP8("v_permlane32_swap_b32", s[0], s[8], s[1], s[9], s[2], s[10], s[3], s[11], s[4], s[12], s[5], s[13],
                 s[6], s[14], s[7], s[15]);
@@ -544,8 +569,23 @@
 int raster_scan_chunks(const RowRanges& rr, uint32_t* pair_off, uint32_t* pair_owner, void* temp, size_t temp_bytes,
                        bool library, hipStream_t st);
 
-__device__ inline float edge_min_q(float a, float b, float c, float d_fixed, float lo, float hi) {
-  const float t = fminf(fmaxf(-(b * d_fixed) * __builtin_amdgcn_rcpf(c), lo), hi);
+__host__ __device__ inline float fast_rcp(float x) {
+#if defined(__HIP_DEVICE_COMPILE__)
+  return __builtin_amdgcn_rcpf(x);
+#else
+  return 1.0f / x;
+#endif
+}
+__host__ __device__ inline float fast_exp(float x) {
+#if defined(__HIP_DEVICE_COMPILE__)
+  return __expf(x);
+#else
+  return expf(x);
+#endif
+}
+
+__host__ __device__ inline float edge_min_q(float a, float b, float c, float d_fixed, float lo, float hi) {
+  const float t = fminf(fmaxf(-(b * d_fixed) * fast_rcp(c), lo), hi);
   const float q0 = a * d_fixed * d_fixed, q1 = 2.f * b * d_fixed * t, q2 = c * t * t;
   return (q0 + q1 + q2) - 2e-5f * (q0 + fabsf(q1) + q2);
 }
@@ -573,5 +613,55 @@
   return m;
 }
 
-}
-}
+__host__ __device__ inline float tile_min_alpha(float mx, float my, float o, float cx, float cy, float cz, float X0, float Y0) {
+  const float x1 = X0 + 15.f, y1 = Y0 + 15.f;
+  if (mx >= X0 && mx <= x1 && my >= Y0 && my <= y1) return 0.f;
+  float qmax = 0.f;
+#pragma unroll
+  for (int c = 0; c < 4; ++c) {
+    const float dx = ((c & 1) ? x1 : X0) - mx, dy = ((c & 2) ? y1 : Y0) - my;
+    const float q0 = cx * dx * dx, q1 = 2.f * cy * dx * dy, q2 = cz * dy * dy;
+    qmax = fmaxf(qmax, (q0 + q1 + q2) + 2e-5f * (q0 + fabsf(q1) + q2));
+  }
+  const float a = fminf(ALPHA_MAX, o * fast_exp(-0.5f * (qmax + 1e-3f)) * (1.f - 1e-5f));
+  if (!(a >= ALPHA_MIN * 1.001f)) return 0.f;
+  const float lx = X0 - mx, hx = x1 - mx, ly = Y0 - my, hy = y1 - my;
+  float m = edge_min_q(cx, cy, cz, lx, ly, hy);
+  m = fminf(m, edge_min_q(cx, cy, cz, hx, ly, hy));
+  m = fminf(m, edge_min_q(cz, cy, cx, ly, lx, hx));
+  m = fminf(m, edge_min_q(cz, cy, cx, hy, lx, hx));
+  if (!(m > 1e-6f)) return 0.f;
+  return a;
+}
+
+struct TileRays {
+  float rx0, rx1, ry0, ry1;
+};
+__host__ __device__ inline TileRays tile_rays(float X0, float Y0, float cxp, float cyp, float fx, float fy) {
+  return TileRays{(X0 - cxp) / fx, ((X0 + 15.f) - cxp) / fx, (Y0 - cyp) / fy, ((Y0 + 15.f) - cyp) / fy};
+}
+__device__ inline TileRays tile_rays_uniform(const TileRays& t) {
+  auto u = [](float v) { return __builtin_bit_cast(float, __builtin_amdgcn_readfirstlane(__builtin_bit_cast(int, v))); };
+  return TileRays{u(t.rx0), u(t.rx1), u(t.ry0), u(t.ry1)};
+}
+constexpr float INTERIOR_DEN_MARGIN = 1e-6f, INTERIOR_D0_MARGIN = 1e-6f;
+__host__ __device__ inline bool blend_interior(float mx, float my, float opacity, float pz, float cx, float cy, float cz,
+                                               float rz, float q, float nx, float ny, float nz, float X0, float Y0,
+                                               const TileRays& t) {
+  if (!(opacity < ALPHA_MAX)) return false;
+  const float ax = fmaxf(fabsf(t.rx0), fabsf(t.rx1)), ay = fmaxf(fabsf(t.ry0), fabsf(t.ry1));
+  const float e_den = INTERIOR_DEN_MARGIN * (fabsf(nx) * ax + fabsf(ny) * ay + fabsf(nz));
+  const float y0 = ny * t.ry0, y1 = ny * t.ry1, x0 = nx * t.rx0, x1 = nx * t.rx1;
+  const float d00 = (x0 + y0) + nz, d10 = (x1 + y0) + nz, d01 = (x0 + y1) + nz, d11 = (x1 + y1) + nz;
+  const float den_max = fmaxf(fmaxf(d00, d10), fmaxf(d01, d11)), den_min = fminf(fminf(d00, d10), fminf(d01, d11));
+  if (!(den_max + e_den < -DEN_EPS)) return false;
+  const float inv_max = fast_rcp(den_max);
+  const float da = q * inv_max, db = q * fast_rcp(den_min);
+  const float dlo = fminf(da, db), dhi = fmaxf(da, db);
+  const float m = fmaxf(fabsf(da), fabsf(db)) * (INTERIOR_D0_MARGIN - e_den * inv_max);
+  if (!(dlo - m > pz - rz && dhi + m < pz + rz)) return false;
+  return tile_min_alpha(mx, my, opacity, cx, cy, cz, X0, Y0) > 0.f;
+}
+
+}
+}
diff --git a/pings_amd/csrc/raster_fwd.hip b/pings_amd/csrc/raster_fwd.hip
--- a/pings_amd/csrc/raster_fwd.hip
+++ b/pings_amd/csrc/raster_fwd.hip
@@ -364,26 +364,6 @@
   }
 }
 
-__device__ inline float tile_min_alpha(float mx, float my, float o, float cx, float cy, float cz, float X0, float Y0) {
-  const float x1 = X0 + 15.f, y1 = Y0 + 15.f;
-  if (mx >= X0 && mx <= x1 && my >= Y0 && my <= y1) return 0.f;
-  float qmax = 0.f;
-#pragma unroll
-  for (int c = 0; c < 4; ++c) {
-    const float dx = ((c & 1) ? x1 : X0) - mx, dy = ((c & 2) ? y1 : Y0) - my;
-    const float q0 = cx * dx * dx, q1 = 2.f * cy * dx * dy, q2 = cz * dy * dy;
-    qmax = fmaxf(qmax, (q0 + q1 + q2) + 2e-5f * (q0 + fabsf(q1) + q2));
-  }
-  const float a = fminf(ALPHA_MAX, o * __expf(-0.5f * (qmax + 1e-3f)) * (1.f - 1e-5f));
-  if (!(a >= ALPHA_MIN * 1.001f)) return 0.f;
-  const float lx = X0 - mx, hx = x1 - mx, ly = Y0 - my, hy = y1 - my;
-  float m = edge_min_q(cx, cy, cz, lx, ly, hy);
-  m = fminf(m, edge_min_q(cx, cy, cz, hx, ly, hy));
-  m = fminf(m, edge_min_q(cz, cy, cx, ly, lx, hx));
-  m = fminf(m, edge_min_q(cz, cy, cx, hy, lx, hx));
-  if (!(m > 1e-6f)) return 0.f;
-  return a;
-}
 
 struct DsRange { uint32_t kmin, shift; };
 
@@ -859,6 +839,19 @@
   return PINGS_OK;
 }
 
+PINGS_API int pings_raster_debug_interior(const float* records, const float* tile_origins, int64_t n, float cxp,
+                                          float cyp, float fx, float fy, uint8_t* flags) {
+  PINGS_ARG_CHECK(n >= 0 && (n == 0 || (records && tile_origins && flags)), "null pointer / negative count");
+  PINGS_ARG_CHECK(fx > 0.f && fy > 0.f, "non-positive focal length");
+  for (int64_t i = 0; i < n; ++i) {
+    const float* r = records + 16 * i;
+    const float X0 = tile_origins[2 * i], Y0 = tile_origins[2 * i + 1];
+    flags[i] = blend_interior(r[0], r[1], r[2], r[3], r[4], r[5], r[6], r[7], r[11], r[12], r[13], r[14], X0, Y0,
+                              tile_rays(X0, Y0, cxp, cyp, fx, fy)) ? 1 : 0;
+  }
+  return PINGS_OK;
+}
+
 PINGS_API int pings_raster_preprocess(const pings_raster_settings* s, int P, const float* means3D,
                                       const float* colors, const float* opacities,
                                       const float* scales, const float* rotations,
diff --git a/pings_amd/csrc/raster_layout.hip b/pings_amd/csrc/raster_layout.hip
--- a/pings_amd/csrc/raster_layout.hip
+++ b/pings_amd/csrc/raster_layout.hip
@@ -151,6 +151,7 @@
   if (const char* e = getenv("PINGS_ROWSUM_WGS")) k.rowsum_wgs = (unsigned)std::min(std::max(atoi(e), 1), 65535);
   if (const char* e = getenv("PINGS_GRAD_FILL")) k.grad_fill_wgs = e[0] == 'l' ? 0u : (unsigned)std::min(std::max(atoi(e), 1), 65535);
   if (const char* e = getenv("PINGS_CHAIN_SUM")) k.chain_sum_lanes = e[0] == 'l';
+  if (const char* e = getenv("PINGS_BLEND_INTERIOR")) k.blend_interior = atoi(e) != 0;
   return k;
 }
 
@@ -164,6 +165,7 @@
   p.seg_on = p.seg > 0 && I > (int64_t)num_tiles * (p.seg / 4) && I > 2 * (int64_t)p.seg;
   p.seg_reuse = p.seg <= 65535u && k.seg_reuse;
   p.long_thr = k.bwd_long;
+  p.interior_bwd = k.blend_interior;
   return p;
 }
 
```

New measurement: 2836 Mpix/s, median of 6. 1.04x the previous value.
